# suyashk12/hipgp

Measured on NVIDIA B200. Metric: toeplitz_matvec_GBps_in_pcg_1e6grid, higher is better.
Workload: dtype f32

## Files before the change

### hipgp_b200/csrc/cols_blk_kernel.cuh

```cuda
#pragma once
#include "fast_kernels.cuh"
#include "tma_maps.cuh"

namespace hipgp {

#ifdef HIPGP_EMU
static inline void nbar_sync(int id, int count) { emu::g_named_barrier[id].sync(count); }
static inline void warp_sync_all() {
    const int tid = (int)(threadIdx.x + blockDim.x * (threadIdx.y + blockDim.y * threadIdx.z));
    emu::g_warp_barrier[tid >> 5].wait();
}
#else
__device__ __forceinline__ void nbar_sync(int id, int count) { asm volatile("bar.sync %0, %1;" ::"r"(id), "r"(count) : "memory"); }
__device__ __forceinline__ void warp_sync_all() { __syncwarp(); }
#endif

template <int GS> __device__ __forceinline__ void blk_sync(int b) {
    if (GS == 32) warp_sync_all(); else nbar_sync(1 + b, GS);
}

template <int R, int S, class T>
__device__ __forceinline__ void blk_fill_pairs(TwPair<T>* dst, const cplx<T>* tab, int tid, int nt) {
    for (int i = tid; i < TwPairs<R>::n * S; i += nt) { const int p = i / S; dst[i] = tw_pair_global<R, S, T>(tab, p, i - p * S); }
}
template <int R, int S, bool SM, class T> __device__ __forceinline__ TwPair<T> blk_pair(const cplx<T>* tab, int p, int j) {
    return SM ? reinterpret_cast<const TwPair<T>*>(tab)[p * S + j] : tw_pair_global<R, S, T>(tab, p, j);
}

template <int R, int S, bool SM, class T>
__device__ __forceinline__ void blk_twiddles(cplx<T>* w, const cplx<T>* tab, int j) {
#pragma unroll
    for (int p = 0; p < TwPairs<R>::n; ++p) {
        const TwPair<T> e = blk_pair<R, S, SM, T>(tab, p, j);
        w[2 * p + 1] = e.a;
        if (2 * p + 2 < R) w[2 * p + 2] = e.b;
    }
}

template <int R, int S, bool SM, bool CONJ, int CH, class T>
__device__ __forceinline__ void blk_twiddle_mul(Lane<T>* v, const cplx<T>* tab, int j) {
    constexpr int PC = CH / 2 > 0 ? CH / 2 : 1;
#pragma unroll
    for (int p0 = 0; p0 < TwPairs<R>::n; p0 += PC) {
        TwPair<T> e[PC];
#pragma unroll
        for (int c = 0; c < PC; ++c) if (p0 + c < TwPairs<R>::n) e[c] = blk_pair<R, S, SM, T>(tab, p0 + c, j);
#pragma unroll
        for (int c = 0; c < PC; ++c) if (p0 + c < TwPairs<R>::n) {
            const int r = 2 * (p0 + c) + 1;
            v[r] = CONJ ? lmulc(v[r], e[c].a) : lmul(v[r], e[c].a);
            if (r + 1 < R) v[r + 1] = CONJ ? lmulc(v[r + 1], e[c].b) : lmul(v[r + 1], e[c].b);
        }
#ifndef HIPGP_EMU
        if (p0 + PC < TwPairs<R>::n) asm volatile("" ::: "memory");
#endif
    }
}

template <class T, int NL, int NT, int MINB, int R0, int R1, int R2>
struct ColsBlkCfg {
    using G = TileGeo<T, NL, R0, R1, R2>;
    static constexpr int Ln = G::Ln, BS = Ln / R0, GS = NT / R0;
    static constexpr int IB2 = (BS / R1) * NL, IB3 = (BS / R2) * NL;
    static constexpr bool ok = (NT % R0 == 0) && (GS % 32 == 0) && (GS == 32 || R0 <= 15) && (IB2 % GS == 0) && (IB3 % GS == 0) &&
                               ((IB2 / GS) * R1 <= 16) && ((IB3 / GS) * R2 <= 16) && (BS % R2 == 0);
    static constexpr size_t tw_bytes = 2 * sizeof(cplx<T>) * (size_t)((R0 / 2) * (Ln / R0) + (R1 / 2) * (BS / R1));
    static constexpr size_t side_bytes = (size_t)(Ln + Ln / R2) * NL * 8;
    static constexpr bool tw_smem = (size_t)MINB * (G::smem_bytes() + side_bytes + tw_bytes + 1024) <= 228 * 1024;
    static constexpr size_t smem_bytes = G::smem_bytes() + side_bytes + (tw_smem ? tw_bytes : 0);
};

template <class T, int NL, int NT, int MINB, int R0, int R1, int R2>
__global__ void __launch_bounds__(NT, MINB) cols_blk_kernel(const HIPGP_GRID_CONSTANT ColsParams<T> P, const HIPGP_GRID_CONSTANT ColsTmaMaps maps) {
    using Cfg = ColsBlkCfg<T, NL, NT, MINB, R0, R1, R2>;
    using G = typename Cfg::G;
    constexpr int Ln = G::Ln, RLAST = R2, LPT = LaneInfo<T>::LPT, TBL = NL * LPT, S0 = Ln / R0;
    constexpr int BS = Cfg::BS, GS = Cfg::GS, S1 = BS / R1;
    constexpr bool TWS = Cfg::tw_smem;
    constexpr int TWCH = R0 >= 16 ? 5 : R0;
    static_assert(Cfg::ok, "radix list / tile shape not usable with block-local middle sections");
    constexpr int LEG0 = G::leg(S0), LEG1 = G::leg(S1);
    constexpr int SPEC_LANE = 8;
    constexpr int SIDE_SLOTS = Ln + Ln / RLAST;
    constexpr int SIDE_LANES = SIDE_SLOTS * NL / 2;
    HIPGP_DYN_SMEM(smem_raw);
    Lane<T>* s = reinterpret_cast<Lane<T>*>(smem_raw);
    unsigned char* side = smem_raw + G::smem_bytes();
    const int tid = threadIdx.x;
    if (P.done_flag && *P.done_flag) return;
    const int blk = tid / GS, u = tid - blk * GS;

    const cplx<T>* tw0 = P.f.twst + P.f.twoff[0];
    const cplx<T>* tw1 = P.f.twst + P.f.twoff[1];
    __shared__ unsigned long long s_bar[3];
    const bool tma_in = P.tma_in != 0, tma_spec = P.tma_spec != 0;
    if ((tma_in || tma_spec) && tid == 0) { tma_bar_init(&s_bar[0]); tma_bar_init(&s_bar[1]); warps_bar_init(&s_bar[2], NT / 32); tma_fence_before_issue(); }
    if (tma_in || tma_spec) __syncthreads();
    if (TWS) {
        TwPair<T>* t0 = reinterpret_cast<TwPair<T>*>(side + Cfg::side_bytes);
        TwPair<T>* t1 = t0 + TwPairs<R0>::n * S0;
        blk_fill_pairs<R0, S0, T>(t0, tw0, tid, NT);
        blk_fill_pairs<R1, S1, T>(t1, tw1, tid, NT);
        tw0 = reinterpret_cast<const cplx<T>*>(t0); tw1 = reinterpret_cast<const cplx<T>*>(t1);
        __syncthreads();
    }

    const int mode = P.mode;
    const size_t pitch = (size_t)P.pitch;
    const size_t spitch = P.spec_pitch ? (size_t)P.spec_pitch : (size_t)P.pitch;
    const long ntiles = (long)P.nx * P.ny * P.nz;
    unsigned tile_bz = 0;
    auto tile_origin = [&](long t, long& c0, size_t& ioff, size_t& ooff) {
        const unsigned tt = (unsigned)t, nx = (unsigned)P.nx, ny = (unsigned)P.ny, nz = (unsigned)P.nz;
        unsigned bx, by, bz;
        if (P.batch_fastest) { bz = tt % nz; const unsigned r = tt / nz; bx = r % nx; by = r / nx; }
        else { bx = tt % nx; const unsigned r = tt / nx; by = r % ny; bz = r / ny; }
        c0 = (long)bx * TBL;
        tile_bz = bz;
        ioff = (size_t)by * P.in_ostride + (size_t)bz * P.in_bstride + c0;
        ooff = (size_t)by * P.out_ostride + (size_t)bz * P.out_bstride + c0;
    };
    auto sslot = [](int p) { return p + (p >> G::LOGRL); };
    const bool spec_smem = P.spec_stage != 0;
    const int n_in = P.n_in, n_out = P.n_out;
    const bool stage_in = P.in_stage != 0;
    const bool zero_hi = is_pow2(R0) && n_in <= Ln / 2;
    const bool out_lo = is_pow2(R0) && n_out <= Ln / 2;
    const size_t rstep = (size_t)S0 * pitch;

    auto prefetch_input = [&](long t) {
        long c0; size_t ioff, ooff;
        tile_origin(t, c0, ioff, ooff);
        const long nvalid = P.inner - c0;
        const cplx<T>* in = P.in + ioff;
        constexpr int NIT = (SIDE_LANES + NT - 1) / NT;
        const int total = n_in * NL;
#pragma unroll
        for (int k = 0; k < NIT; ++k) {
            const int w = tid + k * NT;
            const int i = w / NL, lane = w - i * NL;
            if (w < total && (long)lane * LPT < nvalid) cp_async<16>(side + (size_t)w * 16, in + (size_t)i * pitch + lane * LPT);
        }
        cp_async_commit();
    };

    auto issue_input = [&](long t) {
        long c0; size_t ioff, ooff;
        tile_origin(t, c0, ioff, ooff);
        const unsigned box_bytes = (unsigned)P.tma_in_rows * NL * 16u;
        tma_fence_before_issue();
        tma_bar_expect(&s_bar[0], box_bytes * (unsigned)P.tma_in_nbox);
        for (int k = 0; k < P.tma_in_nbox; ++k)
            tma_load_box3(side + (size_t)k * box_bytes, &maps.in, (int)(2 * c0), k * P.tma_in_rows, (int)tile_bz, &s_bar[0]);
    };
    auto stage_next = [&](long tn) {
        if (tn >= ntiles) return;
        if (tma_in) { if (tid == 0) issue_input(tn); }
        else if (stage_in) prefetch_input(tn);
    };

    stage_next((long)blockIdx.x);
    for (unsigned iter = 0;; ++iter) {
        const long t = (long)blockIdx.x + (long)iter * gridDim.x;
        if (t >= ntiles) break;
        const unsigned ph = iter & 1u;
        long c0; size_t ioff, ooff;
        tile_origin(t, c0, ioff, ooff);
        const long nvalid = P.inner - c0;
        const cplx<T>* in = P.in + ioff;
        cplx<T>* out = P.out + ooff;
        if (tma_in) { tma_bar_wait(&s_bar[0], ph, 8, NT); if (mode != CM_FUSED) __syncthreads(); }
        else { cp_async_wait_all(); __syncthreads(); }

        if (mode != CM_INV) {
#pragma unroll 1
            for (int it = tid; it < S0 * NL; it += NT) {
                const int lane = it % NL, j = it / NL;
                const bool ok = (long)lane * LPT < nvalid;
                Lane<T> v[R0];
                if (tma_in) {
                    const Lane<T>* sp = reinterpret_cast<const Lane<T>*>(side) + (j * NL + lane);
#pragma unroll
                    for (int r = 0; r < R0 / 2; ++r) v[r] = sp[r * S0 * NL];
                    lbfly_zero_hi<R0, T>(v);
                } else if (stage_in) {
                    const Lane<T>* sp = reinterpret_cast<const Lane<T>*>(side) + (j * NL + lane);
                    if (zero_hi) {
#pragma unroll
                        for (int r = 0; r < R0 / 2; ++r) v[r] = (ok && j + r * S0 < n_in) ? sp[r * S0 * NL] : lzero<T>();
                        lbfly_zero_hi<R0, T>(v);
                    } else {
#pragma unroll
                        for (int r = 0; r < R0; ++r) v[r] = (ok && j + r * S0 < n_in) ? sp[r * S0 * NL] : lzero<T>();
                        lbfly<R0, false, T>(v);
                    }
                } else {
                    const cplx<T>* gp = in + (size_t)j * pitch + lane * LPT;
                    if (zero_hi) {
#pragma unroll
                        for (int r = 0; r < R0 / 2; ++r) v[r] = (ok && j + r * S0 < n_in) ? lane_from_global(gp + r * rstep) : lzero<T>();
                        lbfly_zero_hi<R0, T>(v);
                    } else {
#pragma unroll
                        for (int r = 0; r < R0; ++r) v[r] = (ok && j + r * S0 < n_in) ? lane_from_global(gp + r * rstep) : lzero<T>();
                        lbfly<R0, false, T>(v);
                    }
                }
                blk_twiddle_mul<R0, S0, TWS, false, TWCH>(v, tw0, j);
                Lane<T>* base = s + (G::slot(j) * NL + lane);
#pragma unroll
                for (int r = 0; r < R0; ++r) base[r * LEG0] = v[r];
            }
            __syncthreads();
            if (!(mode == CM_FUSED && spec_smem)) stage_next(t + gridDim.x);
        }

        const int pb = blk * BS;
        if (mode == CM_FUSED && spec_smem && tma_spec) {
            if (tid == 0) {
                tma_fence_before_issue();
                tma_bar_expect(&s_bar[1], (unsigned)Cfg::side_bytes);
                tma_load_box3(side, &maps.spec, (int)c0, 0, 0, &s_bar[1]);
            }
        } else if (mode == CM_FUSED && spec_smem) {
            const unsigned char* sp = reinterpret_cast<const unsigned char*>(P.spec) + (size_t)c0 * sizeof(T);
            constexpr int ROWB = NL * SPEC_LANE;
            constexpr int CH = ROWB >= 16 ? 16 : 8, NCH = ROWB / CH;
            constexpr int NIT = (BS * NCH + GS - 1) / GS;
#pragma unroll
            for (int k = 0; k < NIT; ++k) {
                const int w = u + k * GS;
                const int p = pb + w / NCH, c = w % NCH;
                if (w < BS * NCH) cp_async<CH>(side + (size_t)sslot(p) * ROWB + c * CH, sp + (size_t)p * spitch * sizeof(T) + c * CH);
            }
            cp_async_commit();
        }
        if (mode != CM_INV) {
            constexpr int NIT = Cfg::IB2 / GS;
            Lane<T> v[NIT][R1];
            cplx<T> w[NIT][R1];
            Lane<T>* base[NIT];
#pragma unroll
            for (int k = 0; k < NIT; ++k) {
                const int q = u + k * GS;
                const int lane = q % NL, j = q / NL;
                base[k] = s + (G::slot(pb + j) * NL + lane);
                blk_twiddles<R1, S1, TWS>(w[k], tw1, j);
#pragma unroll
                for (int r = 0; r < R1; ++r) v[k][r] = base[k][r * LEG1];
            }
#pragma unroll
            for (int k = 0; k < NIT; ++k) {
                lbfly<R1, false, T>(v[k]);
#pragma unroll
                for (int r = 1; r < R1; ++r) v[k][r] = lmul(v[k][r], w[k][r]);
#pragma unroll
                for (int r = 0; r < R1; ++r) base[k][r * LEG1] = v[k][r];
            }
            if (mode == CM_FUSED && spec_smem) {
                if (tma_spec) tma_bar_wait(&s_bar[1], ph, 9, NT);
                else cp_async_wait_all();
            }
            blk_sync<GS>(blk);
        }
        {
            constexpr int NIT = Cfg::IB3 / GS;
#pragma unroll
            for (int k = 0; k < NIT; ++k) {
                const int q = u + k * GS;
                const int lane = q % NL;
                const bool ok = (long)lane * LPT < nvalid;
                const int p0 = pb + (q / NL) * RLAST;
                Lane<T>* base = s + (G::slot(p0) * NL + lane);
                Lane<T> v[RLAST];
                if (mode == CM_INV) {
                    const cplx<T>* gp = in + cols_rowoff<T>(p0, P.pitch, P.in_split_len, P.in_split_stride) + lane * LPT;
#pragma unroll
                    for (int r = 0; r < RLAST; ++r) v[r] = ok ? lane_from_global(gp + r * pitch) : lzero<T>();
                } else {
#pragma unroll
                    for (int r = 0; r < RLAST; ++r) v[r] = base[r * NL];
                    lbfly<RLAST, false, T>(v);
                }
                if (mode == CM_FUSED) {
                    if (spec_smem) {
                        const unsigned char* sp = side + ((size_t)sslot(p0) * NL + lane) * SPEC_LANE;
#pragma unroll
                        for (int r = 0; r < RLAST; ++r) v[r] = lane_spec_smem(v[r], sp + r * NL * SPEC_LANE);
                    } else if (ok) {
                        const size_t sidx = (size_t)p0 * spitch + c0 + lane * LPT;
#pragma unroll
                        for (int r = 0; r < RLAST; ++r) v[r] = lane_spec(v[r], P.spec, P.spec_kind, sidx + (size_t)r * spitch);
                    }
                }
                if (mode == CM_FWD) {
                    if (ok) {
                        cplx<T>* gp = out + cols_rowoff<T>(p0, P.pitch, P.out_split_len, P.out_split_stride) + lane * LPT;
#pragma unroll
                        for (int r = 0; r < RLAST; ++r) lane_to_global(gp + r * pitch, v[r]);
                    }
                } else {
                    lbfly<RLAST, true, T>(v);
#pragma unroll
                    for (int r = 0; r < RLAST; ++r) base[r * NL] = v[r];
                }
            }
        }
        if (mode == CM_FWD) continue;
        const bool early_in = tma_in && mode == CM_FUSED && spec_smem;
        if (early_in) {
            warp_sync_all();
            if (tid == 0) { warps_bar_arrive_and_wait(&s_bar[2], ph, 10, NT / 32); stage_next(t + gridDim.x); }
            else if ((tid & 31) == 0) warps_bar_arrive(&s_bar[2], 10, NT / 32);
        }
        blk_sync<GS>(blk);
        {
            constexpr int NIT = Cfg::IB2 / GS;
            Lane<T> v[NIT][R1];
            cplx<T> w[NIT][R1];
            Lane<T>* base[NIT];
#pragma unroll
            for (int k = 0; k < NIT; ++k) {
                const int q = u + k * GS;
                const int lane = q % NL, j = q / NL;
                base[k] = s + (G::slot(pb + j) * NL + lane);
                blk_twiddles<R1, S1, TWS>(w[k], tw1, j);
#pragma unroll
                for (int r = 0; r < R1; ++r) v[k][r] = base[k][r * LEG1];
            }
#pragma unroll
            for (int k = 0; k < NIT; ++k) {
#pragma unroll
                for (int r = 1; r < R1; ++r) v[k][r] = lmulc(v[k][r], w[k][r]);
                lbfly<R1, true, T>(v[k]);
#pragma unroll
                for (int r = 0; r < R1; ++r) base[k][r * LEG1] = v[k][r];
            }
        }
        __syncthreads();
        if (mode == CM_FUSED && spec_smem && !early_in) stage_next(t + gridDim.x);
        {
#pragma unroll 1
            for (int it = tid; it < S0 * NL; it += NT) {
                const int lane = it % NL, j = it / NL;
                const bool ok = (long)lane * LPT < nvalid;
                const Lane<T>* base = s + (G::slot(j) * NL + lane);
                Lane<T> v[R0];
#pragma unroll
                for (int r = 0; r < R0; ++r) v[r] = base[r * LEG0];
                blk_twiddle_mul<R0, S0, TWS, true, TWCH>(v, tw0, j);
                cplx<T>* gp = out + (size_t)((unsigned)j * (unsigned)P.pitch + (unsigned)(lane * LPT));
                const unsigned rs = (unsigned)S0 * (unsigned)P.pitch;
                if (out_lo) {
                    lbfly<R0, true, T>(v);
                    if (ok) {
#pragma unroll
                        for (int r = 0; r < R0 / 2; ++r) if (j + r * S0 < n_out) lane_to_global(gp + (size_t)((unsigned)r * rs), v[r]);
                    }
                } else {
                    lbfly<R0, true, T>(v);
                    if (ok) {
#pragma unroll
                        for (int r = 0; r < R0; ++r) if (j + r * S0 < n_out) lane_to_global(gp + (size_t)((unsigned)r * rs), v[r]);
                    }
                }
            }
        }
    }
}

}
```

### hipgp_b200/csrc/conv_kernels.cuh

```cuda
#pragma once
#include "fft_engine.cuh"

namespace hipgp {

enum RowsFwdMode { RF_PLAIN = 0, RF_PUPDATE = 1, RF_XRUPDATE = 2, RF_SELFDOT = 3 };
enum RowsInvMode { RI_PLAIN = 0, RI_DOT = 1 };
enum DotKind { DOT_PAP = 0, DOT_ZR = 1, DOT_RR = 2 };
enum ColsMode { CM_FWD = 0, CM_INV = 1, CM_FUSED = 2 };
enum SpecKind { SPEC_NONE = 0, SPEC_REAL = 1, SPEC_CPLX = 2, SPEC_CPLX_CONJ = 3 };

struct PcgDev {
    double* zr;
    double* zr_prev;
    double* pAp;
    double* rr;
    const double* rr_all;
    double* partial;
    unsigned* row_cnt;
    unsigned* rhs_cnt;
    int* flags;
    double tol;
    int B;
    int cg_mode;
};

template <class T> __device__ __forceinline__ T warp_sum(T v) {
#pragma unroll
    for (int o = 16; o > 0; o >>= 1) v += __shfl_xor_sync(0xffffffffu, v, o);
    return v;
}

__device__ __forceinline__ void pcg_finalize(const PcgDev& st, int kind, long g0, long g1, int nrows, int tid, int nthreads) {
    __shared__ unsigned s_last;
    __shared__ double s_red[32];
    const int b0 = (int)(g0 / nrows), b1 = (int)((g1 - 1) / nrows);
    for (int b = b0; b <= b1; ++b) {
        const long lo = g0 > (long)b * nrows ? g0 : (long)b * nrows;
        const long hi = g1 < (long)(b + 1) * nrows ? g1 : (long)(b + 1) * nrows;
        __syncthreads();
        if (tid == 0) {
            __threadfence();
            const unsigned done = atomicAdd(st.row_cnt + b, (unsigned)(hi - lo)) + (unsigned)(hi - lo);
            s_last = (done == (unsigned)nrows);
        }
        __syncthreads();
        if (!s_last) continue;
        __threadfence();
        double acc = 0.0;
        const volatile double* part = st.partial + (long)b * nrows;
        for (int i = tid; i < nrows; i += nthreads) acc += part[i];
        acc = warp_sum(acc);
        if ((tid & 31) == 0) s_red[tid >> 5] = acc;
        __syncthreads();
        if (tid < 32) {
            double v = tid < (nthreads >> 5) ? s_red[tid] : 0.0;
            v = warp_sum(v);
            if (tid == 0) {
                st.row_cnt[b] = 0;
                if (kind == DOT_PAP) st.pAp[b] = v;
                else if (kind == DOT_ZR) { st.zr_prev[b] = st.zr[b]; st.zr[b] = v; }
                else {
                    st.rr[b] = v;
                    if (st.cg_mode) { st.zr_prev[b] = st.zr[b]; st.zr[b] = v; }
                }
                __threadfence();
                if (kind == DOT_RR) {
                    const unsigned nb = atomicAdd(st.rhs_cnt, 1u) + 1u;
                    if (nb == (unsigned)st.B) {
                        __threadfence();
                        bool all = true;
                        const volatile double* rr = st.rr_all ? st.rr_all : st.rr;
                        for (int i = 0; i < st.B; ++i) all = all && (sqrt(rr[i]) < st.tol);
                        st.rhs_cnt[0] = 0;
                        st.flags[1] += 1;
                        st.flags[2] = 0;
                        if (all) st.flags[0] = 1;
                    }
                }
            }
        }
    }
}

template <class T>
struct RowsParams {
    const T* in;
    T* out;
    T* v0;
    T* v1;
    const T* v2;
    cplx<T>* W;
    long total_rows;
    int nrows;
    int n_real;
    int L, H;
    long W_pitch;
    int W_rows;
    LineFft<T> f;
    const cplx<T>* twL;
    const cplx<T>* twLp;
    const int* part;
    const int* pairq;
    const int* pairs; const cplx<T>* pairw; int npair0;
    const int* quadq; const cplx<T>* quadw; int nquad;
    int RB, RBP;
    int mode, dot_kind, do_fft;
    int vec_ok;
    int vec16_ok;
    int tma_ok;
    int tma_op;
    const void* spec; int spec_kind;
    PcgDev st;
};

template <class T>
__global__ void __launch_bounds__(256) rows_fwd_kernel(RowsParams<T> P) {
    HIPGP_DYN_SMEM(smem_raw);
    cplx<T>* s = reinterpret_cast<cplx<T>*>(smem_raw);
    const int tid = threadIdx.x, nthreads = blockDim.x;
    const int warp = tid >> 5, lane = tid & 31, nwarps = nthreads >> 5;
    if (P.mode != RF_PLAIN && P.st.flags[0]) return;
    const long g0 = (long)blockIdx.x * P.RB;
    const long g1 = g0 + P.RB < P.total_rows ? g0 + P.RB : P.total_rows;
    const int nl = (int)(g1 - g0);
    const int H = P.H, RBP = P.RBP, n = P.n_real;

    for (int line = warp; line < P.RB; line += nwarps) {
        if (line >= nl) {
            if (P.do_fft) for (int k = lane; k < H; k += 32) s[(size_t)k * RBP + line] = mk<T>(0, 0);
            continue;
        }
        const long g = g0 + line;
        const int b = (int)(g / P.nrows);
        const size_t off = (size_t)g * n;
        T acc = 0;
        T coef = 0;
        bool first = false;
        if (P.mode == RF_PUPDATE) {
            first = P.st.flags[2] != 0;
            coef = first ? (T)0 : (T)(P.st.zr[b] / P.st.zr_prev[b]);
        } else if (P.mode == RF_XRUPDATE) {
            coef = (T)(P.st.zr[b] / P.st.pAp[b]);
        }
        for (int k = lane; k < H; k += 32) {
            T e[2];
#pragma unroll
            for (int h = 0; h < 2; ++h) {
                const int i = 2 * k + h;
                T val = 0;
                if (i < n) {
                    if (P.mode == RF_PLAIN) {
                        val = P.in[off + i];
                    } else if (P.mode == RF_PUPDATE) {
                        const T z = P.in[off + i];
                        val = first ? z : z + coef * P.v0[off + i];
                        P.v0[off + i] = val;
                    } else if (P.mode == RF_SELFDOT) {
                        val = P.in[off + i];
                        acc += val * val;
                    } else {
                        const T pv = P.v2[off + i];
                        P.v1[off + i] = P.v1[off + i] + coef * pv;
                        val = P.v0[off + i] - coef * P.in[off + i];
                        P.v0[off + i] = val;
                        acc += val * val;
                    }
                }
                e[h] = val;
            }
            if (P.do_fft) s[(size_t)k * RBP + line] = mk<T>(e[0], e[1]);
        }
        if (P.mode == RF_XRUPDATE || P.mode == RF_SELFDOT) {
            const double tot = warp_sum((double)acc);
            if (lane == 0) P.st.partial[g] = tot;
        }
    }
    if (P.mode == RF_XRUPDATE) pcg_finalize(P.st, DOT_RR, g0, g1, P.nrows, tid, nthreads);
    if (P.mode == RF_SELFDOT) pcg_finalize(P.st, DOT_ZR, g0, g1, P.nrows, tid, nthreads);
    if (!P.do_fft) return;
    __syncthreads();

    fft_forward(s, RBP, P.RB, P.f, tid, nthreads);

    for (int w = tid; w < H * P.RB; w += nthreads) {
        const int line = w % P.RB, p = w / P.RB;
        const int k = P.f.rev[p];
        if (k == 0) {
            const cplx<T> z = s[line];
            s[line] = mk<T>((T)2 * (z.x + z.y), 0);
            s[(size_t)H * RBP + line] = mk<T>((T)2 * (z.x - z.y), 0);
        } else {
            const int k2 = H - k;
            if (k <= k2) {
                const int p2 = P.f.pos[k2];
                const cplx<T> a = s[(size_t)p * RBP + line], c = conj(s[(size_t)p2 * RBP + line]);
                const cplx<T> E = a + c;
                const cplx<T> d = a - c;
                const cplx<T> O = mk<T>(d.y, -d.x);
                const cplx<T> t = P.twL[k] * O;
                s[(size_t)p * RBP + line] = E + t;
                if (k != k2) s[(size_t)p2 * RBP + line] = conj(E - t);
            }
        }
    }
    __syncthreads();

    for (int line = warp; line < nl; line += nwarps) {
        const long g = g0 + line;
        cplx<T>* dst = P.W + ((size_t)(g / P.nrows) * P.W_rows + (g % P.nrows)) * P.W_pitch;
        for (int q = lane; q <= H; q += 32) dst[q] = s[(size_t)q * RBP + line];
    }
}

template <class T>
__device__ __forceinline__ cplx<T> apply_spec(cplx<T> v, const void* spec, int kind, size_t idx) {
    if (kind == SPEC_REAL) return v * reinterpret_cast<const T*>(spec)[idx];
    const cplx<T> sv = reinterpret_cast<const cplx<T>*>(spec)[idx];
    return kind == SPEC_CPLX ? v * sv : mulc(v, sv);
}

template <class T>
__global__ void __launch_bounds__(256) rows_inv_kernel(RowsParams<T> P) {
    HIPGP_DYN_SMEM(smem_raw);
    cplx<T>* s = reinterpret_cast<cplx<T>*>(smem_raw);
    const int tid = threadIdx.x, nthreads = blockDim.x;
    const int warp = tid >> 5, lane = tid & 31, nwarps = nthreads >> 5;
    if (P.mode != RI_PLAIN && P.st.flags[0]) return;
    const long g0 = (long)blockIdx.x * P.RB;
    const long g1 = g0 + P.RB < P.total_rows ? g0 + P.RB : P.total_rows;
    const int nl = (int)(g1 - g0);
    const int H = P.H, RBP = P.RBP, n = P.n_real;

    for (int line = warp; line < P.RB; line += nwarps) {
        if (line >= nl) {
            for (int q = lane; q <= H; q += 32) s[(size_t)q * RBP + line] = mk<T>(0, 0);
            continue;
        }
        const long g = g0 + line;
        const cplx<T>* src = P.W + ((size_t)(g / P.nrows) * P.W_rows + (g % P.nrows)) * P.W_pitch;
        for (int q = lane; q <= H; q += 32) {
            cplx<T> v = src[q];
            if (P.spec_kind != SPEC_NONE) v = apply_spec(v, P.spec, P.spec_kind, (size_t)q);
            s[(size_t)q * RBP + line] = v;
        }
    }
    __syncthreads();

    for (int w = tid; w < H * P.RB; w += nthreads) {
        const int line = w % P.RB, p = w / P.RB;
        const int k = P.f.rev[p];
        if (k == 0) {
            const T y0 = s[line].x, yh = s[(size_t)H * RBP + line].x;
            s[line] = mk<T>(y0 + yh, y0 - yh);
        } else {
            const int k2 = H - k;
            if (k <= k2) {
                const int p2 = P.f.pos[k2];
                const cplx<T> a = s[(size_t)p * RBP + line], c = conj(s[(size_t)p2 * RBP + line]);
                const cplx<T> E = a + c;
                const cplx<T> O = mulc(a - c, P.twL[k]);
                const cplx<T> iO = mk<T>(-O.y, O.x);
                s[(size_t)p * RBP + line] = E + iO;
                if (k != k2) s[(size_t)p2 * RBP + line] = conj(E - iO);
            }
        }
    }
    __syncthreads();

    fft_inverse(s, RBP, P.RB, P.f, tid, nthreads);

    for (int line = warp; line < nl; line += nwarps) {
        const long g = g0 + line;
        const size_t off = (size_t)g * n;
        T acc = 0;
        for (int k = lane; k < H; k += 32) {
            const cplx<T> z = s[(size_t)k * RBP + line];
            const int i = 2 * k;
            if (i < n) { P.out[off + i] = z.x; if (P.mode == RI_DOT) acc += z.x * P.v0[off + i]; }
            if (i + 1 < n) { P.out[off + i + 1] = z.y; if (P.mode == RI_DOT) acc += z.y * P.v0[off + i + 1]; }
        }
        if (P.mode == RI_DOT) {
            const double tot = warp_sum((double)acc);
            if (lane == 0) P.st.partial[g] = tot;
        }
    }
    if (P.mode == RI_DOT) pcg_finalize(P.st, P.dot_kind, g0, g1, P.nrows, tid, nthreads);
}

template <class T>
struct ColsParams {
    const cplx<T>* in;
    cplx<T>* out;
    int n_in, n_out;
    long inner;
    long pitch;
    long in_ostride, in_bstride, out_ostride, out_bstride;
    LineFft<T> f;
    int TB, TBP;
    int mode;
    const void* spec; int spec_kind;
    long spec_pitch;
    int spec_stage;
    int in_stage;
    int nx, ny, nz;
    int tma_in, tma_in_rows, tma_in_nbox;
    int tma_spec;
    int batch_fastest;
    const int* done_flag;
    int out_split_len; long out_split_stride;
    int in_split_len; long in_split_stride;
};
template <class T> __device__ __forceinline__ size_t cols_rowoff(int i, long pitch, int split_len, long split_stride) {
    return split_len ? (size_t)(i / split_len) * split_stride + (size_t)(i % split_len) * pitch : (size_t)i * pitch;
}

template <class T>
__global__ void __launch_bounds__(512) cols_pass_kernel(ColsParams<T> P) {
    HIPGP_DYN_SMEM(smem_raw);
    cplx<T>* s = reinterpret_cast<cplx<T>*>(smem_raw);
    const int tid = threadIdx.x, nthreads = blockDim.x;
    if (P.done_flag && *P.done_flag) return;
    const long c0 = (long)blockIdx.x * P.TB;
    const int nc = (int)(P.inner - c0 < P.TB ? P.inner - c0 : P.TB);
    const int L = P.f.Ln, TB = P.TB, TBP = P.TBP;
    const cplx<T>* in = P.in + (size_t)blockIdx.y * P.in_ostride + (size_t)blockIdx.z * P.in_bstride + c0;
    cplx<T>* out = P.out + (size_t)blockIdx.y * P.out_ostride + (size_t)blockIdx.z * P.out_bstride + c0;

    const int rows_in = P.mode == CM_INV ? L : P.n_in;
    for (int w = tid; w < L * TB; w += nthreads) {
        const int c = w % TB, i = w / TB;
        cplx<T> v = mk<T>(0, 0);
        if (i < rows_in && c < nc) v = in[cols_rowoff<T>(i, P.pitch, P.in_split_len, P.in_split_stride) + c];
        s[(size_t)i * TBP + c] = v;
    }
    __syncthreads();

    if (P.mode != CM_INV) fft_forward(s, TBP, TB, P.f, tid, nthreads);
    if (P.mode == CM_FUSED) {
        for (int w = tid; w < L * TB; w += nthreads) {
            const int c = w % TB, i = w / TB;
            if (c < nc) s[(size_t)i * TBP + c] = apply_spec(s[(size_t)i * TBP + c], P.spec, P.spec_kind, (size_t)i * (P.spec_pitch ? P.spec_pitch : P.pitch) + c0 + c);
        }
        __syncthreads();
    }
    if (P.mode != CM_FWD) fft_inverse(s, TBP, TB, P.f, tid, nthreads);

    const int rows_out = P.mode == CM_FWD ? L : P.n_out;
    for (int w = tid; w < rows_out * TB; w += nthreads) {
        const int c = w % TB, i = w / TB;
        if (c < nc) out[cols_rowoff<T>(i, P.pitch, P.out_split_len, P.out_split_stride) + c] = s[(size_t)i * TBP + c];
    }
}


}
```

### hipgp_b200/csrc/cuda_emu.h

```cpp
#pragma once
#ifdef HIPGP_EMU
#include <algorithm>
#include <atomic>
#include <cmath>
#include <condition_variable>
#include <cstdint>
#include <cstdio>
#include <cstdlib>
#include <cstring>
#include <functional>
#include <mutex>
#include <thread>
#include <vector>

#define __global__
#define __device__
#define __host__
#define __forceinline__ inline
#define __restrict__
#define __launch_bounds__(...)
#define __shared__ static
#define __align__(n) alignas(n)

struct uint3e { unsigned x, y, z; };
struct dim3 {
    unsigned x, y, z;
    dim3(unsigned x_ = 1, unsigned y_ = 1, unsigned z_ = 1) : x(x_), y(y_), z(z_) {}
};
struct float2 { float x, y; };
struct double2 { double x, y; };
static inline float2 make_float2(float a, float b) { return float2{a, b}; }
static inline double2 make_double2(double a, double b) { return double2{a, b}; }

typedef void* cudaStream_t;
typedef void* cudaEvent_t;
typedef int cudaError_t;
enum { cudaSuccess = 0 };
enum cudaMemcpyKind { cudaMemcpyHostToDevice, cudaMemcpyDeviceToHost, cudaMemcpyDeviceToDevice, cudaMemcpyDefault };

namespace emu {
struct Barrier {
    std::mutex mu;
    std::condition_variable cv;
    int expected = 0, arrived = 0;
    unsigned long gen = 0;
    void reset(int n) { expected = n; arrived = 0; }
    void wait() {
        std::unique_lock<std::mutex> lk(mu);
        unsigned long g = gen;
        if (++arrived >= expected) { arrived = 0; ++gen; cv.notify_all(); return; }
        cv.wait(lk, [&] { return gen != g; });
    }
    void drop() {
        std::unique_lock<std::mutex> lk(mu);
        --expected;
        if (expected > 0 && arrived >= expected) { arrived = 0; ++gen; cv.notify_all(); }
    }
};
struct NamedBarrier {
    std::mutex mu;
    std::condition_variable cv;
    int arrived = 0;
    unsigned long gen = 0;
    void reset() { arrived = 0; }
    void arrive(int expected) {
        std::unique_lock<std::mutex> lk(mu);
        if (++arrived >= expected) { arrived = 0; ++gen; cv.notify_all(); }
    }
    void sync(int expected) {
        std::unique_lock<std::mutex> lk(mu);
        const unsigned long g = gen;
        if (++arrived >= expected) { arrived = 0; ++gen; cv.notify_all(); return; }
        cv.wait(lk, [&] { return gen != g; });
    }
};
extern NamedBarrier g_named_barrier[16];
extern thread_local dim3 t_threadIdx, t_blockIdx;
extern dim3 g_blockDim, g_gridDim;
extern Barrier g_block_barrier;
extern Barrier g_warp_barrier[64];
extern unsigned char* g_dyn_smem;
extern double g_shfl_scratch[64][32][2];

template <class F>
void launch(dim3 grid, dim3 block, size_t smem, F&& body) {
    const int T = (int)(block.x * block.y * block.z);
    g_blockDim = block; g_gridDim = grid;
    std::vector<unsigned char> dyn(smem + 64);
    g_dyn_smem = dyn.data() + (64 - ((uintptr_t)dyn.data() & 63)) % 64;
    Barrier start, finish;
    const long nblocks = (long)grid.x * grid.y * grid.z;
    start.reset(T); finish.reset(T);
    auto worker = [&](int t) {
        t_threadIdx = dim3(t % block.x, (t / block.x) % block.y, t / (block.x * block.y));
        for (long b = 0; b < nblocks; ++b) {
            t_blockIdx = dim3((unsigned)(b % grid.x), (unsigned)((b / grid.x) % grid.y), (unsigned)(b / ((long)grid.x * grid.y)));
            if (t == 0) {
                g_block_barrier.reset(T);
                for (int w = 0; w < 64; ++w) g_warp_barrier[w].reset(32);
                for (int w = 0; w < 16; ++w) g_named_barrier[w].reset();
            }
            start.wait();
            body();
            g_block_barrier.drop();
            finish.wait();
        }
    };
    std::vector<std::thread> th;
    th.reserve(T);
    for (int t = 1; t < T; ++t) th.emplace_back(worker, t);
    worker(0);
    for (auto& x : th) x.join();
    g_dyn_smem = nullptr;
}
}

#define threadIdx emu::t_threadIdx
#define blockIdx emu::t_blockIdx
#define blockDim emu::g_blockDim
#define gridDim emu::g_gridDim
static inline void __syncthreads() { emu::g_block_barrier.wait(); }
static inline void __syncwarp(unsigned = 0xffffffffu) {}
static inline void __threadfence() { std::atomic_thread_fence(std::memory_order_seq_cst); }

template <class T>
static inline T __shfl_xor_sync(unsigned, T v, int lanemask) {
    const int tid = (int)(threadIdx.x + blockDim.x * (threadIdx.y + blockDim.y * threadIdx.z));
    const int w = tid >> 5, l = tid & 31;
    static_assert(sizeof(T) <= 16, "shfl payload");
    std::memcpy(emu::g_shfl_scratch[w][l], &v, sizeof(T));
    emu::g_warp_barrier[w].wait();
    T r;
    std::memcpy(&r, emu::g_shfl_scratch[w][l ^ lanemask], sizeof(T));
    emu::g_warp_barrier[w].wait();
    return r;
}
template <class T>
static inline T __shfl_down_sync(unsigned, T v, int delta) {
    const int tid = (int)(threadIdx.x + blockDim.x * (threadIdx.y + blockDim.y * threadIdx.z));
    const int w = tid >> 5, l = tid & 31;
    std::memcpy(emu::g_shfl_scratch[w][l], &v, sizeof(T));
    emu::g_warp_barrier[w].wait();
    T r;
    std::memcpy(&r, emu::g_shfl_scratch[w][(l + delta) < 32 ? l + delta : l], sizeof(T));
    emu::g_warp_barrier[w].wait();
    return r;
}
static inline unsigned atomicAdd(unsigned* p, unsigned v) { return __atomic_fetch_add(p, v, __ATOMIC_SEQ_CST); }
static inline int atomicAdd(int* p, int v) { return __atomic_fetch_add(p, v, __ATOMIC_SEQ_CST); }
static inline unsigned atomicInc_emu(unsigned* p) { return __atomic_fetch_add(p, 1u, __ATOMIC_SEQ_CST); }
template <class T> static inline T __ldg(const T* p) { return *p; }
static inline int __popc(int x) { return __builtin_popcount((unsigned)x); }
static inline void sincospi(double x, double* s, double* c) { *s = std::sin(M_PI * x); *c = std::cos(M_PI * x); }
static inline double cospi(double x) { return std::cos(M_PI * x); }
static inline double rsqrt(double x) { return 1.0 / std::sqrt(x); }
static inline float rsqrtf(float x) { return 1.0f / std::sqrt(x); }

static inline cudaError_t cudaMalloc(void** p, size_t n) { *p = std::malloc(n ? n : 1); return *p ? 0 : 2; }
static inline cudaError_t cudaFree(void* p) { std::free(p); return 0; }
static inline cudaError_t cudaMallocHost(void** p, size_t n) { return cudaMalloc(p, n); }
static inline cudaError_t cudaFreeHost(void* p) { return cudaFree(p); }
static inline cudaError_t cudaMemcpyAsync(void* d, const void* s, size_t n, cudaMemcpyKind, cudaStream_t) { std::memcpy(d, s, n); return 0; }
static inline cudaError_t cudaMemcpy(void* d, const void* s, size_t n, cudaMemcpyKind) { std::memcpy(d, s, n); return 0; }
static inline cudaError_t cudaMemsetAsync(void* d, int v, size_t n, cudaStream_t) { std::memset(d, v, n); return 0; }
static inline cudaError_t cudaMemset(void* d, int v, size_t n) { std::memset(d, v, n); return 0; }
static inline cudaError_t cudaStreamSynchronize(cudaStream_t) { return 0; }
static inline cudaError_t cudaDeviceSynchronize() { return 0; }
static inline cudaError_t cudaGetLastError() { return 0; }
static inline cudaError_t cudaSetDevice(int) { return 0; }
static inline cudaError_t cudaGetDevice(int* d) { *d = 0; return 0; }
static inline const char* cudaGetErrorString(cudaError_t) { return "emu"; }

#define HIPGP_DYN_SMEM(name) unsigned char* name = emu::g_dyn_smem
#define HIPGP_LAUNCH(kernel, grid, block, smem, stream, ...) \
    emu::launch((grid), (block), (smem), [&]() { kernel(__VA_ARGS__); })
#define HIPGP_SET_MAX_SMEM(kernel, bytes) ((void)0)

#else
#include <cuda_runtime.h>
#include <cstdint>
#include <cstdio>
#include <cstdlib>
#include <cstring>
#include <cmath>
#include <algorithm>
#include <vector>

#define HIPGP_DYN_SMEM(name) extern __shared__ __align__(128) unsigned char name[]
#define HIPGP_LAUNCH(kernel, grid, block, smem, stream, ...) \
    kernel<<<(grid), (block), (smem), (stream)>>>(__VA_ARGS__)
#define HIPGP_SET_MAX_SMEM(kernel, bytes) \
    cudaFuncSetAttribute(kernel, cudaFuncAttributeMaxDynamicSharedMemorySize, (int)(bytes))
#endif
```

### hipgp_b200/csrc/fast_kernels.cuh

```cuda
#pragma once
#include "lane_fft.cuh"

namespace hipgp {

template <class T> __device__ __forceinline__ void ld2(const T* p, bool vec, T& a, T& b, bool ok0, bool ok1) {
    if (vec && ok1) { const cplx<T> t = ld_stream(reinterpret_cast<const cplx<T>*>(p)); a = t.x; b = t.y; }
    else { a = ok0 ? ld_stream(p) : (T)0; b = ok1 ? ld_stream(p + 1) : (T)0; }
}
template <class T> __device__ __forceinline__ void st2(T* p, bool vec, T a, T b, bool ok0, bool ok1) {
    if (vec && ok1) { st_stream(reinterpret_cast<cplx<T>*>(p), mk<T>(a, b)); }
    else { if (ok0) st_stream(p, a); if (ok1) st_stream(p + 1, b); }
}

__device__ __forceinline__ double team_sum(double v, int tw) {
    for (int o = tw >> 1; o > 0; o >>= 1) v += __shfl_xor_sync(0xffffffffu, v, o);
    return v;
}

__device__ __forceinline__ Lane<float> lane_spec(Lane<float> v, const void* spec, int kind, size_t idx) {
    if (kind == SPEC_REAL) {
        const cplx<float> sv = ld_stream(reinterpret_cast<const cplx<float>*>(reinterpret_cast<const float*>(spec) + idx));
        return lmul_real2(v, sv.x, sv.y);
    }
    const cplx<float>* sp = reinterpret_cast<const cplx<float>*>(spec) + idx;
    const cplx<float> w0 = ld_stream(sp), w1 = ld_stream(sp + 1);
    return kind == SPEC_CPLX ? lmul_cplx2<false>(v, w0, w1) : lmul_cplx2<true>(v, w0, w1);
}
__device__ __forceinline__ Lane<double> lane_spec(Lane<double> v, const void* spec, int kind, size_t idx) {
    if (kind == SPEC_REAL) return lscale(v, ld_stream(reinterpret_cast<const double*>(spec) + idx));
    const cplx<double> w = ld_stream(reinterpret_cast<const cplx<double>*>(spec) + idx);
    return kind == SPEC_CPLX ? lmul(v, w) : lmulc(v, w);
}
__device__ __forceinline__ Lane<float> lane_spec_smem(Lane<float> v, const void* p) {
    const float2 s2 = *reinterpret_cast<const float2*>(p);
    Lane<float> r; r.re = __fmul2_rn(v.re, s2); r.im = __fmul2_rn(v.im, s2); return r;
}
__device__ __forceinline__ Lane<double> lane_spec_smem(Lane<double> v, const void* p) { return lscale(v, *reinterpret_cast<const double*>(p)); }

template <class T, int NL, int NT, int MINB, int R0, int... Rs>
__global__ void __launch_bounds__(NT, MINB) cols_fast_kernel(ColsParams<T> P) {
    using G = TileGeo<T, NL, R0, Rs...>;
    constexpr int Ln = G::Ln, NST = G::NST, RLAST = G::RLAST, LPT = LaneInfo<T>::LPT, TBL = NL * LPT, S0 = Ln / R0;
    HIPGP_DYN_SMEM(smem_raw);
    Lane<T>* s = reinterpret_cast<Lane<T>*>(smem_raw);
    const int tid = threadIdx.x;
    if (P.done_flag && *P.done_flag) return;
    const int mode = P.mode;
    const size_t pitch = (size_t)P.pitch;
    const size_t spitch = P.spec_pitch ? (size_t)P.spec_pitch : (size_t)P.pitch;
    const long ntiles = (long)P.nx * P.ny * P.nz;
    auto tile_origin = [&](long t, long& c0, size_t& ioff, size_t& ooff) {
        long bx, by, bz;
        if (P.batch_fastest) { bz = t % P.nz; const long r = t / P.nz; bx = r % P.nx; by = r / P.nx; }
        else { bx = t % P.nx; const long r = t / P.nx; by = r % P.ny; bz = r / P.ny; }
        c0 = bx * TBL;
        ioff = (size_t)by * P.in_ostride + (size_t)bz * P.in_bstride + c0;
        ooff = (size_t)by * P.out_ostride + (size_t)bz * P.out_bstride + c0;
    };

    if constexpr (NST == 1) {
        for (long t = blockIdx.x; t < ntiles; t += gridDim.x) {
            long c0; size_t ioff, ooff;
            tile_origin(t, c0, ioff, ooff);
            const long nvalid = P.inner - c0;
            const cplx<T>* in = P.in + ioff;
            cplx<T>* out = P.out + ooff;
            for (int lane = tid; lane < NL; lane += NT) {
                if ((long)lane * LPT >= nvalid) continue;
                const int rows_in = mode == CM_INV ? Ln : P.n_in;
                const int rows_out = mode == CM_FWD ? Ln : P.n_out;
                Lane<T> v[R0];
#pragma unroll
                for (int r = 0; r < R0; ++r)
                    v[r] = r < rows_in ? lane_from_global(in + cols_rowoff<T>(r, P.pitch, P.in_split_len, P.in_split_stride) + lane * LPT) : lzero<T>();
                if (mode != CM_INV) lbfly<R0, false, T>(v);
                if (mode == CM_FUSED) {
#pragma unroll
                    for (int r = 0; r < R0; ++r) v[r] = lane_spec(v[r], P.spec, P.spec_kind, (size_t)r * spitch + c0 + lane * LPT);
                }
                if (mode != CM_FWD) lbfly<R0, true, T>(v);
#pragma unroll
                for (int r = 0; r < R0; ++r)
                    if (r < rows_out) lane_to_global(out + cols_rowoff<T>(r, P.pitch, P.out_split_len, P.out_split_stride) + lane * LPT, v[r]);
            }
        }
        return;
    } else {
        constexpr int LEG0 = G::leg(S0);
        constexpr int SPEC_LANE = 8;
        constexpr int SIDE_SLOTS = Ln + Ln / RLAST;
        constexpr int SIDE_LANES = SIDE_SLOTS * NL / 2;
        unsigned char* side = smem_raw + G::smem_bytes();
        auto sslot = [](int p) { return p + (p >> G::LOGRL); };
        const cplx<T>* tw0 = P.f.twst + P.f.twoff[0];
        const bool spec_smem = P.spec_stage != 0;
        const int n_in = P.n_in, n_out = P.n_out;
        const bool stage_in = P.in_stage != 0;
        const bool zero_hi = is_pow2(R0) && n_in <= Ln / 2;
        const bool out_lo = is_pow2(R0) && n_out <= Ln / 2;
        const size_t rstep = (size_t)S0 * pitch;

        auto prefetch_input = [&](long t) {
            long c0; size_t ioff, ooff;
            tile_origin(t, c0, ioff, ooff);
            const long nvalid = P.inner - c0;
            const cplx<T>* in = P.in + ioff;
            constexpr int NIT = (SIDE_LANES + NT - 1) / NT;
            const int total = n_in * NL;
#pragma unroll
            for (int k = 0; k < NIT; ++k) {
                const int w = tid + k * NT;
                const int i = w / NL, lane = w - i * NL;
                if (w < total && (long)lane * LPT < nvalid) cp_async<16>(side + (size_t)w * 16, in + (size_t)i * pitch + lane * LPT);
            }
            cp_async_commit();
        };

        long t = blockIdx.x;
        if (stage_in && t < ntiles) prefetch_input(t);
        for (; t < ntiles; t += gridDim.x) {
            long c0; size_t ioff, ooff;
            tile_origin(t, c0, ioff, ooff);
            const long nvalid = P.inner - c0;
            const cplx<T>* in = P.in + ioff;
            cplx<T>* out = P.out + ooff;
            cp_async_wait_all();
            __syncthreads();

            if (mode != CM_INV) {
#pragma unroll 1
                for (int it = tid; it < S0 * NL; it += NT) {
                    const int lane = it % NL, j = it / NL;
                    const bool ok = (long)lane * LPT < nvalid;
                    cplx<T> w[R0];
                    lane_twiddles<R0, S0>(w, tw0, j);
                    Lane<T> v[R0];
                    if (stage_in) {
                        const Lane<T>* sp = reinterpret_cast<const Lane<T>*>(side) + (j * NL + lane);
                        if (zero_hi) {
#pragma unroll
                            for (int r = 0; r < R0 / 2; ++r) v[r] = (ok && j + r * S0 < n_in) ? sp[r * S0 * NL] : lzero<T>();
                            lbfly_zero_hi<R0, T>(v);
                        } else {
#pragma unroll
                            for (int r = 0; r < R0; ++r) v[r] = (ok && j + r * S0 < n_in) ? sp[r * S0 * NL] : lzero<T>();
                            lbfly<R0, false, T>(v);
                        }
                    } else {
                        const cplx<T>* gp = in + (size_t)j * pitch + lane * LPT;
                        if (zero_hi) {
#pragma unroll
                            for (int r = 0; r < R0 / 2; ++r) v[r] = (ok && j + r * S0 < n_in) ? lane_from_global(gp + r * rstep) : lzero<T>();
                            lbfly_zero_hi<R0, T>(v);
                        } else {
#pragma unroll
                            for (int r = 0; r < R0; ++r) v[r] = (ok && j + r * S0 < n_in) ? lane_from_global(gp + r * rstep) : lzero<T>();
                            lbfly<R0, false, T>(v);
                        }
                    }
#pragma unroll
                    for (int r = 1; r < R0; ++r) v[r] = lmul(v[r], w[r]);
                    Lane<T>* base = s + (G::slot(j) * NL + lane);
#pragma unroll
                    for (int r = 0; r < R0; ++r) base[r * LEG0] = v[r];
                }
                __syncthreads();
                if (spec_smem) {
                    const unsigned char* sp = reinterpret_cast<const unsigned char*>(P.spec) + (size_t)c0 * sizeof(T);
                    constexpr int ROWB = NL * SPEC_LANE;
                    constexpr int CH = ROWB >= 16 ? 16 : 8, NCH = ROWB / CH;
                    constexpr int NIT = (Ln * NCH + NT - 1) / NT;
#pragma unroll
                    for (int k = 0; k < NIT; ++k) {
                        const int w = tid + k * NT;
                        const int p = w / NCH, c = w - p * NCH;
                        if (w < Ln * NCH) cp_async<CH>(side + (size_t)sslot(p) * ROWB + c * CH, sp + (size_t)p * spitch * sizeof(T) + c * CH);
                    }
                    cp_async_commit();
                }
                LaneMidFwd<G, T, NL, NT, Ln / R0, 1, Rs...>::run(s, P.f, tid);
                if (spec_smem) { cp_async_wait_all(); __syncthreads(); }
            }

            {
#pragma unroll 2
                for (int it = tid; it < (Ln / RLAST) * NL; it += NT) {
                    const int lane = it % NL, bf = it / NL;
                    const bool ok = (long)lane * LPT < nvalid;
                    const int p0 = bf * RLAST;
                    Lane<T>* base = s + (G::slot(p0) * NL + lane);
                    Lane<T> v[RLAST];
                    if (mode == CM_INV) {
                        const cplx<T>* gp = in + cols_rowoff<T>(p0, P.pitch, P.in_split_len, P.in_split_stride) + lane * LPT;
#pragma unroll
                        for (int r = 0; r < RLAST; ++r) v[r] = ok ? lane_from_global(gp + r * pitch) : lzero<T>();
                    } else {
#pragma unroll
                        for (int r = 0; r < RLAST; ++r) v[r] = base[r * NL];
                        lbfly<RLAST, false, T>(v);
                    }
                    if (mode == CM_FUSED) {
                        if (spec_smem) {
                            const unsigned char* sp = side + ((size_t)sslot(p0) * NL + lane) * SPEC_LANE;
#pragma unroll
                            for (int r = 0; r < RLAST; ++r) v[r] = lane_spec_smem(v[r], sp + r * NL * SPEC_LANE);
                        } else if (ok) {
                            const size_t sidx = (size_t)p0 * spitch + c0 + lane * LPT;
#pragma unroll
                            for (int r = 0; r < RLAST; ++r) v[r] = lane_spec(v[r], P.spec, P.spec_kind, sidx + (size_t)r * spitch);
                        }
                    }
                    if (mode == CM_FWD) {
                        if (ok) {
                            cplx<T>* gp = out + cols_rowoff<T>(p0, P.pitch, P.out_split_len, P.out_split_stride) + lane * LPT;
#pragma unroll
                            for (int r = 0; r < RLAST; ++r) lane_to_global(gp + r * pitch, v[r]);
                        }
                    } else {
                        lbfly<RLAST, true, T>(v);
#pragma unroll
                        for (int r = 0; r < RLAST; ++r) base[r * NL] = v[r];
                    }
                }
                __syncthreads();
            }
            if (stage_in && t + gridDim.x < ntiles) prefetch_input(t + gridDim.x);
            if (mode == CM_FWD) continue;

            LaneMidInv<G, T, NL, NT, Ln / R0, 1, Rs...>::run(s, P.f, tid);
            {
#pragma unroll 1
                for (int it = tid; it < S0 * NL; it += NT) {
                    const int lane = it % NL, j = it / NL;
                    const bool ok = (long)lane * LPT < nvalid;
                    cplx<T> w[R0];
                    lane_twiddles<R0, S0>(w, tw0, j);
                    const Lane<T>* base = s + (G::slot(j) * NL + lane);
                    Lane<T> v[R0];
#pragma unroll
                    for (int r = 0; r < R0; ++r) v[r] = base[r * LEG0];
#pragma unroll
                    for (int r = 1; r < R0; ++r) v[r] = lmulc(v[r], w[r]);
                    cplx<T>* gp = out + (size_t)j * pitch + lane * LPT;
                    lbfly<R0, true, T>(v);
                    if (ok) {
                        if (out_lo) {
#pragma unroll
                            for (int r = 0; r < R0 / 2; ++r) if (j + r * S0 < n_out) lane_to_global(gp + r * rstep, v[r]);
                        } else {
#pragma unroll
                            for (int r = 0; r < R0; ++r) if (j + r * S0 < n_out) lane_to_global(gp + r * rstep, v[r]);
                        }
                    }
                }
            }
        }
    }
}

struct __align__(8) QuadIdx { int a, b; };

template <class T, int NL, int NT, int MINB, int R0, int... Rs>
__global__ void __launch_bounds__(NT, MINB) rows_fwd_fast_kernel(RowsParams<T> P) {
    using G = TileGeo<T, NL, R0, Rs...>;
    constexpr int H = G::Ln, NST = G::NST, RLAST = G::RLAST, LPT = LaneInfo<T>::LPT, NROW = NL * LPT, S0 = H / R0;
    constexpr int LEG0 = G::leg(NST > 1 ? S0 : 1);
    HIPGP_DYN_SMEM(smem_raw);
    Lane<T>* s = reinterpret_cast<Lane<T>*>(smem_raw);
    const int tid = threadIdx.x;
    if (P.mode != RF_PLAIN && P.st.flags[0]) return;
    const long g0 = (long)blockIdx.x * NROW;
    const long g1 = g0 + NROW < P.total_rows ? g0 + NROW : P.total_rows;
    const int nl = (int)(g1 - g0);
    const int n = P.n_real;
    const int mode = P.mode;
    const bool vec = ((n & 1) == 0) && P.vec_ok;
    const bool first_it = (mode == RF_PUPDATE) && (P.st.flags[2] != 0);
    const bool want_dot = (mode == RF_XRUPDATE || mode == RF_SELFDOT);
    __shared__ T s_coef[32];
    __shared__ long s_wbase[32];
    __shared__ double s_part[32];
    if (tid < NROW && tid < nl) {
        const long gr = g0 + tid;
        const long b = gr / P.nrows;
        s_wbase[tid] = (b * P.W_rows + (gr - b * P.nrows)) * P.W_pitch;
        T coef = 0;
        if (mode == RF_PUPDATE) coef = first_it ? (T)0 : (T)(P.st.zr[b] / P.st.zr_prev[b]);
        else if (mode == RF_XRUPDATE) coef = (T)(P.st.zr[b] / P.st.pAp[b]);
        s_coef[tid] = coef;
    }
    __syncthreads();

    const int SROW = (n + 3) & ~3;
    T* side = reinterpret_cast<T*>(smem_raw + G::smem_bytes());
    bool streamed = false;
#ifndef HIPGP_EMU
    bool bulk_store_pending = false;
    if (P.tma_ok && P.vec16_ok && SROW == n && (mode == RF_PLAIN || mode == RF_SELFDOT || P.tma_op)) {
        constexpr int CH = 16 / (int)sizeof(T);
        __shared__ __align__(8) unsigned long long s_mbar;
        const unsigned bytes = (unsigned)((size_t)nl * n * sizeof(T));
        const size_t goff = (size_t)g0 * n;
        T* bufA = reinterpret_cast<T*>(smem_raw);
        T* bufB = bufA + (size_t)NROW * SROW;
        const bool two = mode == RF_PUPDATE && !first_it, three = mode == RF_XRUPDATE;
        if (tid == 0) { mbar_init(&s_mbar, 1); fence_proxy_async(); }
        __syncthreads();
        if (tid == 0) {
            mbar_arrive_expect_tx(&s_mbar, bytes * (three ? 3u : (two ? 2u : 1u)));
            bulk_g2s(side, P.in + goff, bytes, &s_mbar);
            if (two) bulk_g2s(bufA, (const T*)P.v0 + goff, bytes, &s_mbar);
            if (three) { bulk_g2s(bufA, (const T*)P.v0 + goff, bytes, &s_mbar); bulk_g2s(bufB, P.v2 + goff, bytes, &s_mbar); }
        }
        constexpr int NW = NT / 32, WPR = NW > NROW ? NW / NROW : 1;
        constexpr int tws = WPR > 1 ? 32 : (H / CH >= 32 ? 32 : (H / CH >= 16 ? 16 : (H / CH >= 8 ? 8 : 4)));
        constexpr int rpw = 32 / tws, TW = WPR > 1 ? 32 * WPR : tws, rstep = WPR > 1 ? NW / WPR : NW * rpw;
        const int warp = tid >> 5, l32 = tid & 31;
        const int ln = WPR > 1 ? l32 + 32 * (warp % WPR) : l32 % tws;
        const int nch = n / CH;
        mbar_wait(&s_mbar, 0);
        if (mode != RF_PLAIN && !(mode == RF_PUPDATE && first_it)) {
            for (int rbase = WPR > 1 ? warp / WPR : warp * rpw; rbase < nl; rbase += rstep) {
                const int row = rbase + (WPR > 1 ? 0 : l32 / tws);
                const bool ractive = row < nl;
                double acc = 0.0;
                if (ractive) {
                    T* srow = side + (size_t)row * SROW;
                    const T* arow = bufA + (size_t)row * SROW;
                    const T* brow = bufB + (size_t)row * SROW;
                    const size_t off = goff + (size_t)row * n;
                    const T coef = s_coef[row];
                    if (three) {
                        constexpr int BS = 4;
                        for (int cb = ln; cb < nch; cb += TW * BS) {
                            Vec16<T> xv[BS];
#pragma unroll
                            for (int k = 0; k < BS; ++k) { const int c = cb + TW * k; if (c < nch) xv[k] = ldv_stream((const T*)P.v1 + off + (size_t)c * CH); }
#pragma unroll
                            for (int k = 0; k < BS; ++k) {
                                const int c = cb + TW * k;
                                if (c < nch) {
                                    Vec16<T> q = *reinterpret_cast<const Vec16<T>*>(srow + c * CH);
                                    const Vec16<T> rv = *reinterpret_cast<const Vec16<T>*>(arow + c * CH);
                                    const Vec16<T> pv = *reinterpret_cast<const Vec16<T>*>(brow + c * CH);
#pragma unroll
                                    for (int e = 0; e < CH; ++e) { xv[k].v[e] = xv[k].v[e] + coef * pv.v[e]; q.v[e] = rv.v[e] - coef * q.v[e]; acc += (double)(q.v[e] * q.v[e]); }
                                    stv_stream(P.v1 + off + (size_t)c * CH, xv[k]);
                                    *reinterpret_cast<Vec16<T>*>(srow + c * CH) = q;
                                }
                            }
                        }
                    } else if (two) {
                        for (int c = ln; c < nch; c += TW) {
                            Vec16<T> z = *reinterpret_cast<const Vec16<T>*>(srow + c * CH);
                            const Vec16<T> pv = *reinterpret_cast<const Vec16<T>*>(arow + c * CH);
#pragma unroll
                            for (int e = 0; e < CH; ++e) z.v[e] = z.v[e] + coef * pv.v[e];
                            *reinterpret_cast<Vec16<T>*>(srow + c * CH) = z;
                        }
                    } else {
                        for (int c = ln; c < nch; c += TW) {
                            const Vec16<T> z = *reinterpret_cast<const Vec16<T>*>(srow + c * CH);
#pragma unroll
                            for (int e = 0; e < CH; ++e) acc += (double)(z.v[e] * z.v[e]);
                        }
                    }
                }
                if (want_dot) {
                    acc = team_sum(acc, WPR > 1 ? 32 : tws);
                    if (ractive && (WPR > 1 ? l32 == 0 : ln == 0)) s_part[row * WPR + warp % WPR] = acc;
                }
            }
        }
        if (mode == RF_PUPDATE || mode == RF_XRUPDATE) {
            fence_proxy_async();
            __syncthreads();
            if (tid == 0) {
                asm volatile("cp.async.bulk.global.shared::cta.bulk_group [%0], [%1], %2;" ::"l"(P.v0 + goff), "r"((unsigned)__cvta_generic_to_shared(side)), "r"(bytes) : "memory");
                asm volatile("cp.async.bulk.commit_group;" ::: "memory");
            }
            bulk_store_pending = true;
        }
        if (want_dot) {
            __syncthreads();
            if (tid < nl) { double a = 0.0; for (int k = 0; k < WPR; ++k) a += s_part[tid * WPR + k]; P.st.partial[g0 + tid] = a; }
        }
        streamed = true;
    }
#endif
    if (!streamed) {
        constexpr int CH = 16 / (int)sizeof(T);
        constexpr int NW = NT / 32, WPR = NW > NROW ? NW / NROW : 1;
        const bool chunked = P.vec16_ok && (n % CH == 0);
        constexpr int tws = WPR > 1 ? 32 : (H / CH >= 32 ? 32 : (H / CH >= 16 ? 16 : (H / CH >= 8 ? 8 : 4)));
        constexpr int rpw = 32 / tws;
        constexpr int TW = WPR > 1 ? 32 * WPR : tws;
        const int warp = tid >> 5, l32 = tid & 31;
        const int ln = WPR > 1 ? l32 + 32 * (warp % WPR) : l32 % tws;
        constexpr int rstep = WPR > 1 ? NW / WPR : NW * rpw;
        for (int rbase = WPR > 1 ? warp / WPR : warp * rpw; rbase < nl; rbase += rstep) {
            const int row = rbase + (WPR > 1 ? 0 : l32 / tws);
            const bool ractive = row < nl;
            T* srow = side + (size_t)(ractive ? row : 0) * SROW;
            const size_t off = (size_t)(g0 + (ractive ? row : 0)) * n;
            const T coef = s_coef[ractive ? row : 0];
            double acc = 0.0;
            if (!ractive) {
            } else if (chunked) {
                const int nch = n / CH;
                auto finish = [&](int c, Vec16<T> a) {
                    if (want_dot) {
#pragma unroll
                        for (int k = 0; k < CH; ++k) acc += (double)(a.v[k] * a.v[k]);
                    }
                    *reinterpret_cast<Vec16<T>*>(srow + c * CH) = a;
                };
#define HIPGP_PIPE(LOAD, PROC)                                                                              \
                {                                                                                           \
                    const int step = TW * BS;                                                               \
                    int cb = ln;                                                                            \
                    LOAD(0, cb);                                                                            \
                    for (; cb < nch; cb += 2 * step) {                                                      \
                        if (cb + step < nch) { LOAD(1, cb + step); }                                        \
                        PROC(0, cb);                                                                        \
                        if (cb + 2 * step < nch) { LOAD(0, cb + 2 * step); }                                \
                        if (cb + step < nch) { PROC(1, cb + step); }                                        \
                    }                                                                                       \
                }
                if (mode == RF_XRUPDATE) {
                    constexpr int BS = 1;
                    Vec16<T> a[2][BS], pv[2][BS], xv[2][BS], rv[2][BS];
#define HIPGP_LD(S, CB)                                                                                     \
                    _Pragma("unroll") for (int k = 0; k < BS; ++k) {                                        \
                        const int c = (CB) + TW * k;                                                        \
                        if (c < nch) {                                                                      \
                            const size_t o = off + (size_t)c * CH;                                          \
                            a[S][k] = ldv_stream(P.in + o); pv[S][k] = ldv_stream(P.v2 + o);                \
                            xv[S][k] = ldv_stream((const T*)P.v1 + o); rv[S][k] = ldv_stream((const T*)P.v0 + o); \
                        }                                                                                   \
                    }
#define HIPGP_PR(S, CB)                                                                                     \
                    _Pragma("unroll") for (int k = 0; k < BS; ++k) {                                        \
                        const int c = (CB) + TW * k;                                                        \
                        if (c < nch) {                                                                      \
                            const size_t o = off + (size_t)c * CH;                                          \
                            _Pragma("unroll") for (int e = 0; e < CH; ++e) {                                \
                                xv[S][k].v[e] = xv[S][k].v[e] + coef * pv[S][k].v[e];                       \
                                a[S][k].v[e] = rv[S][k].v[e] - coef * a[S][k].v[e];                         \
                            }                                                                               \
                            stv_stream(P.v1 + o, xv[S][k]);                                                 \
                            stv_stream(P.v0 + o, a[S][k]);                                                  \
                            finish(c, a[S][k]);                                                             \
                        }                                                                                   \
                    }
                    HIPGP_PIPE(HIPGP_LD, HIPGP_PR)
#undef HIPGP_LD
#undef HIPGP_PR
                } else if (mode == RF_PUPDATE && !first_it) {
                    constexpr int BS = 2;
                    Vec16<T> a[2][BS], pv[2][BS];
#define HIPGP_LD(S, CB)                                                                                     \
                    _Pragma("unroll") for (int k = 0; k < BS; ++k) {                                        \
                        const int c = (CB) + TW * k;                                                        \
                        if (c < nch) { const size_t o = off + (size_t)c * CH; a[S][k] = ldv_stream(P.in + o); pv[S][k] = ldv_stream((const T*)P.v0 + o); } \
                    }
#define HIPGP_PR(S, CB)                                                                                     \
                    _Pragma("unroll") for (int k = 0; k < BS; ++k) {                                        \
                        const int c = (CB) + TW * k;                                                        \
                        if (c < nch) {                                                                      \
                            _Pragma("unroll") for (int e = 0; e < CH; ++e) a[S][k].v[e] = a[S][k].v[e] + coef * pv[S][k].v[e]; \
                            stv_stream(P.v0 + off + (size_t)c * CH, a[S][k]);                               \
                            finish(c, a[S][k]);                                                             \
                        }                                                                                   \
                    }
                    HIPGP_PIPE(HIPGP_LD, HIPGP_PR)
#undef HIPGP_LD
#undef HIPGP_PR
                } else {
                    constexpr int BS = 4;
                    const bool wr = mode == RF_PUPDATE;
                    Vec16<T> a[2][BS];
#define HIPGP_LD(S, CB)                                                                                     \
                    _Pragma("unroll") for (int k = 0; k < BS; ++k) { const int c = (CB) + TW * k; if (c < nch) a[S][k] = ldv_stream(P.in + off + (size_t)c * CH); }
#define HIPGP_PR(S, CB)                                                                                     \
                    _Pragma("unroll") for (int k = 0; k < BS; ++k) {                                        \
                        const int c = (CB) + TW * k;                                                        \
                        if (c < nch) { if (wr) stv_stream(P.v0 + off + (size_t)c * CH, a[S][k]); finish(c, a[S][k]); } \
                    }
                    HIPGP_PIPE(HIPGP_LD, HIPGP_PR)
#undef HIPGP_LD
#undef HIPGP_PR
                }
#undef HIPGP_PIPE
            } else {
                for (int i = ln; i < n; i += TW) {
                    const size_t o = off + i;
                    T a = ld_stream(P.in + o);
                    if (mode == RF_PUPDATE) {
                        if (!first_it) a = a + coef * ld_stream((const T*)P.v0 + o);
                        st_stream(P.v0 + o, a);
                    } else if (mode == RF_XRUPDATE) {
                        const T pv = ld_stream(P.v2 + o);
                        st_stream(P.v1 + o, ld_stream((const T*)P.v1 + o) + coef * pv);
                        a = ld_stream((const T*)P.v0 + o) - coef * a;
                        st_stream(P.v0 + o, a);
                    }
                    if (want_dot) acc += (double)(a * a);
                    srow[i] = a;
                }
            }
            if (ractive) for (int i = n + ln; i < SROW; i += TW) srow[i] = (T)0;
            if (want_dot) {
                acc = team_sum(acc, WPR > 1 ? 32 : tws);
                if (ractive && (WPR > 1 ? l32 == 0 : ln == 0)) s_part[row * WPR + warp % WPR] = acc;
            }
        }
        if (want_dot) {
            __syncthreads();
            if (tid < nl) { double a = 0.0; for (int k = 0; k < WPR; ++k) a += s_part[tid * WPR + k]; P.st.partial[g0 + tid] = a; }
        }
    }
    __syncthreads();
    if (want_dot) pcg_finalize(P.st, mode == RF_XRUPDATE ? DOT_RR : DOT_ZR, g0, g1, P.nrows, tid, NT);

    {
        const bool zero_hi = is_pow2(R0) && R0 > 1 && (n + 1) / 2 <= H / 2;
        const cplx<T>* tw0 = P.f.twst + P.f.twoff[0];
#pragma unroll 1
        for (int it = tid; it < S0 * NL; it += NT) {
            const int lane = it % NL, j = it / NL;
            cplx<T> w[R0];
            if (NST > 1) lane_twiddles<R0, S0>(w, tw0, j);
            const T* srow0 = side + (size_t)(lane * LPT) * SROW;
            const T* srow1 = side + (size_t)(lane * LPT + LPT - 1) * SROW;
            const bool ok0 = lane * LPT < nl, ok1 = lane * LPT + LPT - 1 < nl;
            auto elem = [&](int r) -> Lane<T> {
                const int i = 2 * (j + r * S0);
                const bool in_row = i < SROW;
                const cplx<T> e0 = (ok0 && in_row) ? *reinterpret_cast<const cplx<T>*>(srow0 + i) : mk<T>(0, 0);
                const cplx<T> e1 = (LPT == 2 && ok1 && in_row) ? *reinterpret_cast<const cplx<T>*>(srow1 + i) : mk<T>(0, 0);
                return lane_make(e0, e1);
            };
            Lane<T> v[R0];
            if (zero_hi) {
#pragma unroll
                for (int r = 0; r < R0 / 2; ++r) v[r] = elem(r);
                lbfly_zero_hi<R0, T>(v);
            } else {
#pragma unroll
                for (int r = 0; r < R0; ++r) v[r] = elem(r);
                lbfly<R0, false, T>(v);
            }
            if (NST > 1) {
#pragma unroll
                for (int r = 1; r < R0; ++r) v[r] = lmul(v[r], w[r]);
            }
            Lane<T>* base = s + (G::slot(j) * NL + lane);
#pragma unroll
            for (int r = 0; r < R0; ++r) base[r * LEG0] = v[r];
        }
    }
    __syncthreads();

    if constexpr (NST > 1) {
        LaneMidFwd<G, T, NL, NT, H / R0, 1, Rs...>::run(s, P.f, tid);
        lane_stage<G, T, NL, NT, RLAST, RLAST, false>(s, P.f.twst, tid);
        __syncthreads();
    }

    constexpr int NPAIR0 = NST > 1 ? RLAST / 2 + 1 : H / 2 + 1;
    constexpr int NQUAD = NST > 1 ? (H - RLAST) / 4 : 0;
#pragma unroll 1
    for (int it = tid; it < NPAIR0 * NL; it += NT) {
        const int lane = it % NL, pi = it / NL;
        const QuadIdx pq = reinterpret_cast<const QuadIdx*>(P.pairs)[pi];
        const int q = pq.a, q2 = pq.b;
        Lane<T> Xa, Xb;
        bool two;
        if (q == 0) {
            const Lane<T> z = s[lane];
            Lane<T> zs; zs.re = z.im; zs.im = z.re;
            Xa = lscale(z + zs, (T)2); Xb = lscale(z - zs, (T)2);
            Xa.im = lzero<T>().im; Xb.im = lzero<T>().im;
            two = true;
        } else {
            const cplx<T> wq = ldg_c(P.pairw + pi);
            const Lane<T> a = s[G::slot(q) * NL + lane], c = lconj(s[G::slot(q2) * NL + lane]);
            const Lane<T> E = a + c;
            const Lane<T> t = lmul(lmi<false>(a - c), wq);
            Xa = E + t; Xb = lconj(E - t);
            two = q2 != q;
        }
#pragma unroll
        for (int l = 0; l < LPT; ++l) {
            const int row = lane * LPT + l;
            if (row < nl) {
                cplx<T>* dst = P.W + s_wbase[row];
                WRow<T>::store1(dst, q, lane_get(Xa, l));
                if (two) WRow<T>::store1(dst, q2, lane_get(Xb, l));
            }
        }
    }
    if constexpr (NQUAD > 0) {
        constexpr int QIT = (NQUAD * NL + NT - 1) / NT;
        QuadIdx qq[QIT]; cplx<T> wa[QIT], wa1[QIT];
#pragma unroll
        for (int k = 0; k < QIT; ++k) {
            const int it = tid + k * NT, qi = it / NL;
            if (it < NQUAD * NL) { qq[k] = reinterpret_cast<const QuadIdx*>(P.quadq)[qi]; wa[k] = ldg_c(P.quadw + 2 * qi); wa1[k] = ldg_c(P.quadw + 2 * qi + 1); }
        }
#pragma unroll
        for (int k = 0; k < QIT; ++k) {
            const int it = tid + k * NT, lane = it % NL;
            if (it < NQUAD * NL) {
                const Lane<T>* pa = s + (G::slot(qq[k].a) * NL + lane);
                const Lane<T>* pb = s + (G::slot(qq[k].b) * NL + lane);
                const Lane<T> za = pa[0], za1 = pa[NL], zb = pb[0], zb1 = pb[NL];
                Lane<T> c = lconj(zb1);
                Lane<T> E = za + c;
                Lane<T> t = lmul(lmi<false>(za - c), wa[k]);
                const Lane<T> Xa = E + t, Xb1 = lconj(E - t);
                c = lconj(zb);
                E = za1 + c;
                t = lmul(lmi<false>(za1 - c), wa1[k]);
                const Lane<T> Xa1 = E + t, Xb = lconj(E - t);
                const bool self = qq[k].a == qq[k].b;
#pragma unroll
                for (int l = 0; l < LPT; ++l) {
                    const int row = lane * LPT + l;
                    if (row < nl) {
                        cplx<T>* dst = P.W + s_wbase[row];
                        if (self) WRow<T>::store2(dst, qq[k].a, lane_get(Xa, l), lane_get(Xb1, l));
                        else { WRow<T>::store2(dst, qq[k].a, lane_get(Xa, l), lane_get(Xa1, l)); WRow<T>::store2(dst, qq[k].b, lane_get(Xb, l), lane_get(Xb1, l)); }
                    }
                }
            }
        }
    }
#ifndef HIPGP_EMU
    if (bulk_store_pending && tid == 0) asm volatile("cp.async.bulk.wait_group.read 0;" ::: "memory");
#endif
}

template <class T, int NL, int NT, int MINB, int R0, int... Rs>
__global__ void __launch_bounds__(NT, MINB) rows_inv_fast_kernel(RowsParams<T> P) {
    using G = TileGeo<T, NL, R0, Rs...>;
    constexpr int H = G::Ln, NST = G::NST, RLAST = G::RLAST, LPT = LaneInfo<T>::LPT, NROW = NL * LPT, S0 = H / R0;
    constexpr int LEG0 = G::leg(NST > 1 ? S0 : 1);
    HIPGP_DYN_SMEM(smem_raw);
    Lane<T>* s = reinterpret_cast<Lane<T>*>(smem_raw);
    const int tid = threadIdx.x;
    if (P.mode != RI_PLAIN && P.st.flags[0]) return;
    const long g0 = (long)blockIdx.x * NROW;
    const long g1 = g0 + NROW < P.total_rows ? g0 + NROW : P.total_rows;
    const int nl = (int)(g1 - g0);
    const int n = P.n_real;

    __shared__ long s_wbase[32];
    __shared__ double s_part[32];
    if (tid < NROW && tid < nl) {
        const long gr = g0 + tid;
        const long b = gr / P.nrows;
        s_wbase[tid] = (b * P.W_rows + (gr - b * P.nrows)) * P.W_pitch;
    }
    __syncthreads();

    const int spec_kind = P.spec_kind;
    constexpr int NPAIR0 = NST > 1 ? RLAST / 2 + 1 : H / 2 + 1;
    constexpr int NQUAD = NST > 1 ? (H - RLAST) / 4 : 0;
#pragma unroll 1
    for (int it = tid; it < NPAIR0 * NL; it += NT) {
        const int lane = it % NL, pi = it / NL;
        const QuadIdx pq = reinterpret_cast<const QuadIdx*>(P.pairs)[pi];
        const int q = pq.a, q2 = pq.b;
        const cplx<T> wq = ldg_c(P.pairw + pi);
        cplx<T> ya[LPT], yc[LPT];
#pragma unroll
        for (int l = 0; l < LPT; ++l) {
            const int row = lane * LPT + l;
            ya[l] = mk<T>(0, 0); yc[l] = mk<T>(0, 0);
            if (row < nl) {
                const cplx<T>* src = P.W + s_wbase[row];
                ya[l] = WRow<T>::load1(src, q); yc[l] = WRow<T>::load1(src, q2);
                if (spec_kind != SPEC_NONE) { ya[l] = apply_spec(ya[l], P.spec, spec_kind, (size_t)q); yc[l] = apply_spec(yc[l], P.spec, spec_kind, (size_t)q2); }
            }
        }
        const Lane<T> a = lane_make(ya[0], ya[LPT - 1]);
        Lane<T> c = lane_make(yc[0], yc[LPT - 1]);
        if (q == 0) {
            Lane<T> z; z.re = (a + c).re; z.im = (a - c).re;
            s[lane] = z;
        } else {
            c = lconj(c);
            const Lane<T> E = a + c;
            const Lane<T> iO = lmi<true>(lmulc(a - c, wq));
            s[G::slot(q) * NL + lane] = E + iO;
            if (q2 != q) s[G::slot(q2) * NL + lane] = lconj(E - iO);
        }
    }
    if constexpr (NQUAD > 0) {
        constexpr int QIT = (NQUAD * NL + NT - 1) / NT;
        QuadIdx qq[QIT]; cplx<T> wa[QIT], wa1[QIT];
        cplx<T> ya[QIT][LPT], ya1[QIT][LPT], yb[QIT][LPT], yb1[QIT][LPT];
#pragma unroll
        for (int k = 0; k < QIT; ++k) {
            int it = tid + k * NT;
            it = it < NQUAD * NL ? it : NQUAD * NL - 1;
            const int qi = it / NL;
            qq[k] = reinterpret_cast<const QuadIdx*>(P.quadq)[qi]; wa[k] = ldg_c(P.quadw + 2 * qi); wa1[k] = ldg_c(P.quadw + 2 * qi + 1);
        }
#pragma unroll
        for (int k = 0; k < QIT; ++k) {
            int it = tid + k * NT;
            it = it < NQUAD * NL ? it : NQUAD * NL - 1;
            const int lane = it % NL;
#pragma unroll
            for (int l = 0; l < LPT; ++l) {
                const int row = lane * LPT + l;
                const cplx<T>* src = P.W + s_wbase[row < nl ? row : nl - 1];
                WRow<T>::load2(src, qq[k].a, ya[k][l], ya1[k][l]);
                WRow<T>::load2(src, qq[k].b, yb[k][l], yb1[k][l]);
            }
        }
#pragma unroll
        for (int k = 0; k < QIT; ++k) {
            const int it = tid + k * NT, lane = it % NL;
            if (it < NQUAD * NL) {
                const bool self = qq[k].a == qq[k].b;
                if (spec_kind != SPEC_NONE) {
#pragma unroll
                    for (int l = 0; l < LPT; ++l) {
                        ya[k][l] = apply_spec(ya[k][l], P.spec, spec_kind, (size_t)qq[k].a); ya1[k][l] = apply_spec(ya1[k][l], P.spec, spec_kind, (size_t)qq[k].a + 1);
                        yb[k][l] = apply_spec(yb[k][l], P.spec, spec_kind, (size_t)qq[k].b); yb1[k][l] = apply_spec(yb1[k][l], P.spec, spec_kind, (size_t)qq[k].b + 1);
                    }
                }
                const Lane<T> A = lane_make(ya[k][0], ya[k][LPT - 1]), A1 = lane_make(ya1[k][0], ya1[k][LPT - 1]);
                const Lane<T> Bn = lane_make(yb[k][0], yb[k][LPT - 1]), B1 = lane_make(yb1[k][0], yb1[k][LPT - 1]);
                Lane<T>* pa = s + (G::slot(qq[k].a) * NL + lane);
                Lane<T>* pb = s + (G::slot(qq[k].b) * NL + lane);
                Lane<T> c = lconj(B1);
                Lane<T> E = A + c;
                Lane<T> iO = lmi<true>(lmulc(A - c, wa[k]));
                pa[0] = E + iO;
                pb[NL] = lconj(E - iO);
                if (!self) {
                    c = lconj(Bn);
                    E = A1 + c;
                    iO = lmi<true>(lmulc(A1 - c, wa1[k]));
                    pa[NL] = E + iO;
                    pb[0] = lconj(E - iO);
                }
            }
        }
    }
    __syncthreads();

    if constexpr (NST > 1) {
        lane_stage<G, T, NL, NT, RLAST, RLAST, true>(s, P.f.twst, tid);
        __syncthreads();
        LaneMidInv<G, T, NL, NT, H / R0, 1, Rs...>::run(s, P.f, tid);
    }

    const int SROW = (n + 3) & ~3;
    T* side = reinterpret_cast<T*>(smem_raw + G::smem_bytes());
    const bool want_dot = P.mode == RI_DOT;
    {
        const bool out_lo = is_pow2(R0) && R0 > 1 && (n + 1) / 2 <= H / 2;
        const cplx<T>* tw0 = P.f.twst + P.f.twoff[0];
#pragma unroll 1
        for (int it = tid; it < S0 * NL; it += NT) {
            const int lane = it % NL, j = it / NL;
            cplx<T> w[R0];
            if (NST > 1) lane_twiddles<R0, S0>(w, tw0, j);
            const Lane<T>* base = s + (G::slot(j) * NL + lane);
            Lane<T> v[R0];
#pragma unroll
            for (int r = 0; r < R0; ++r) v[r] = base[r * LEG0];
            if (NST > 1) {
#pragma unroll
                for (int r = 1; r < R0; ++r) v[r] = lmulc(v[r], w[r]);
            }
            lbfly<R0, true, T>(v);
            T* srow0 = side + (size_t)(lane * LPT) * SROW;
            T* srow1 = side + (size_t)(lane * LPT + LPT - 1) * SROW;
            auto put = [&](int r) {
                const int i = 2 * (j + r * S0);
                if (i < SROW) {
                    *reinterpret_cast<cplx<T>*>(srow0 + i) = lane_get(v[r], 0);
                    if (LPT == 2) *reinterpret_cast<cplx<T>*>(srow1 + i) = lane_get(v[r], LPT - 1);
                }
            };
            if (out_lo) {
#pragma unroll
                for (int r = 0; r < R0 / 2; ++r) put(r);
            } else {
#pragma unroll
                for (int r = 0; r < R0; ++r) put(r);
            }
        }
    }
#ifndef HIPGP_EMU
    const bool tma_any = P.tma_ok && P.vec16_ok && SROW == n;
    const bool tma_out = !want_dot && tma_any;
    const bool tma_dot = want_dot && tma_any;
    if (tma_any) fence_proxy_async();
#else
    const bool tma_out = false, tma_dot = false;
#endif
    __syncthreads();
#ifndef HIPGP_EMU
    if (tma_out) {
        if (tid == 0) bulk_s2g(P.out + (size_t)g0 * n, side, (unsigned)((size_t)nl * n * sizeof(T)));
        return;
    }
    if (tma_dot && tid == 0) bulk_s2g_issue(P.out + (size_t)g0 * n, side, (unsigned)((size_t)nl * n * sizeof(T)));
#endif
    {
        constexpr int CH = 16 / (int)sizeof(T);
        constexpr int NW = NT / 32, WPR = NW > NROW ? NW / NROW : 1;
        const bool chunked = P.vec16_ok && (n % CH == 0);
        constexpr int tws = WPR > 1 ? 32 : (H / CH >= 32 ? 32 : (H / CH >= 16 ? 16 : (H / CH >= 8 ? 8 : 4)));
        constexpr int rpw = 32 / tws;
        constexpr int TW = WPR > 1 ? 32 * WPR : tws;
        const int warp = tid >> 5, l32 = tid & 31;
        const int ln = WPR > 1 ? l32 + 32 * (warp % WPR) : l32 % tws;
        constexpr int rstep = WPR > 1 ? NW / WPR : NW * rpw;
        for (int rbase = WPR > 1 ? warp / WPR : warp * rpw; rbase < nl; rbase += rstep) {
            const int row = rbase + (WPR > 1 ? 0 : l32 / tws);
            const bool ractive = row < nl;
            const T* srow = side + (size_t)(ractive ? row : 0) * SROW;
            const size_t off = (size_t)(g0 + (ractive ? row : 0)) * n;
            double acc = 0.0;
            if (!ractive) {
            } else if (chunked) {
                const int nch = n / CH;
                constexpr int BS = 8;
                for (int cb = ln; cb < nch; cb += TW * BS) {
                    Vec16<T> ov[BS];
                    if (want_dot) {
#pragma unroll
                        for (int k = 0; k < BS; ++k) { const int c = cb + TW * k; if (c < nch) ov[k] = ldv_stream((const T*)P.v0 + off + (size_t)c * CH); }
                    }
#pragma unroll
                    for (int k = 0; k < BS; ++k) {
                        const int c = cb + TW * k;
                        if (c < nch) {
                            const Vec16<T> y = *reinterpret_cast<const Vec16<T>*>(srow + c * CH);
                            if (want_dot) {
#pragma unroll
                                for (int e = 0; e < CH; ++e) acc += (double)(y.v[e] * ov[k].v[e]);
                            }
                            if (!tma_dot) stv_stream(P.out + off + (size_t)c * CH, y);
                        }
                    }
                }
            } else if (sizeof(T) == 4 && (n & 1) == 0 && P.vec_ok) {
                for (int c = ln; c < n / 2; c += TW) {
                    const cplx<T> y = *reinterpret_cast<const cplx<T>*>(srow + 2 * c);
                    if (want_dot) {
                        const cplx<T> ov = ld_stream(reinterpret_cast<const cplx<T>*>((const T*)P.v0 + off + 2 * c));
                        acc += (double)(y.x * ov.x) + (double)(y.y * ov.y);
                    }
                    st_stream(reinterpret_cast<cplx<T>*>(P.out + off + 2 * c), y);
                }
            } else {
                for (int i = ln; i < n; i += TW) {
                    const T y = srow[i];
                    if (want_dot) acc += (double)(y * ld_stream((const T*)P.v0 + off + i));
                    st_stream(P.out + off + i, y);
                }
            }
            if (want_dot) {
                acc = team_sum(acc, WPR > 1 ? 32 : tws);
                if (ractive && (WPR > 1 ? l32 == 0 : ln == 0)) s_part[row * WPR + warp % WPR] = acc;
            }
        }
    }
#ifndef HIPGP_EMU
    if (tma_dot && tid == 0) bulk_s2g_wait();
#endif
    if (want_dot) {
        __syncthreads();
        constexpr int WPR2 = (NT / 32) > NROW ? (NT / 32) / NROW : 1;
        if (tid < nl) { double a = 0.0; for (int k = 0; k < WPR2; ++k) a += s_part[tid * WPR2 + k]; P.st.partial[g0 + tid] = a; }
        pcg_finalize(P.st, P.dot_kind, g0, g1, P.nrows, tid, NT);
    }
}

}
```

### hipgp_b200/csrc/plan.cu

```cuda
#include "plan_types.cuh"
#include "setup_kernels.cuh"
#include "kxu_kernels.cuh"

namespace hipgp {
thread_local std::string g_err;
bool g_no_fast = false;
}

namespace hipgp {

template <class T> struct Tag {};
static Geom<float>& geom(hipgp_plan* p, bool wide, Tag<float>) { return wide ? p->gw32 : p->gn32; }
static Geom<double>& geom(hipgp_plan* p, bool wide, Tag<double>) { return wide ? p->gw64 : p->gn64; }

template <class T> static size_t rows_smem(int H, int RBP) { return sizeof(cplx<T>) * (size_t)(H + 1) * RBP; }

template <class T>
static void pick_rows_tiling(long total_rows, int H, int* RB, int* RBP, int* nthreads) {
    int rb = 8;
    while (rb > 1 && (rows_smem<T>(H, rb + 1) > 96 * 1024 || total_rows < (long)rb * 148)) rb >>= 1;
    if (rows_smem<T>(H, rb + 1) > 200 * 1024) throw Error("row axis too long for the shared-memory FFT (L = " + std::to_string(2 * H) + ")");
    *RB = rb; *RBP = rb == 1 ? 1 : rb + 1;
    long work = (long)H * rb / 8;
    *nthreads = work >= 256 ? 256 : (work >= 128 ? 128 : (work >= 64 ? 64 : 32));
}

template <class T> static bool aligned2(const void* p) { return ((uintptr_t)p % (2 * sizeof(T))) == 0; }

template <class T>
static bool launch_rows_fast(hipgp_plan* pl, bool inverse, RowsParams<T>& P, cudaStream_t st) {
    if (g_no_fast) return false;
    switch (P.H) {
#define X(LEN, ...) case LEN: launch_rows_fast_len<T, LEN>(pl, inverse, P, st); return true;
        HIPGP_FAST_LIST(X)
#undef X
        default: return false;
    }
}

template <class T>
static bool geom_allows_fast(const Geom<T>& g) {
    if (sizeof(T) == 8) return true;
    if (g_no_fast || fast_radices(g.H).empty()) return false;
    for (int d = 0; d + 1 < g.D; ++d) if (fast_radices(g.L[d]).empty()) return false;
    return true;
}

template <class T>
static void launch_rows(hipgp_plan* pl, bool inverse, RowsParams<T>& P, cudaStream_t st, bool allow_fast = true) {
    P.vec_ok = (aligned2<T>(P.in) && aligned2<T>(P.out) && aligned2<T>(P.v0) && aligned2<T>(P.v1) && aligned2<T>(P.v2)) ? 1 : 0;
    {
        auto a16 = [](const void* q) { return ((uintptr_t)q % 16) == 0; };
        P.vec16_ok = (a16(P.in) && a16(P.out) && a16(P.v0) && a16(P.v1) && a16(P.v2)) ? 1 : 0;
    }
    if (allow_fast && P.do_fft && launch_rows_fast<T>(pl, inverse, P, st)) return;
    int nth;
    pick_rows_tiling<T>(P.total_rows, P.H, &P.RB, &P.RBP, &nth);
    const size_t smem = rows_smem<T>(P.H, P.RBP);
    dim3 grid((unsigned)((P.total_rows + P.RB - 1) / P.RB));
    PROF_BEGIN(pl, inverse ? 2 : 0, st);
    if (inverse) {
        auto k = rows_inv_kernel<T>;
        if (smem > 48 * 1024) HIPGP_SET_MAX_SMEM(k, smem);
        HIPGP_LAUNCH(k, grid, dim3(nth), smem, st, P);
    } else {
        auto k = rows_fwd_kernel<T>;
        if (smem > 48 * 1024) HIPGP_SET_MAX_SMEM(k, smem);
        HIPGP_LAUNCH(k, grid, dim3(nth), smem, st, P);
    }
    PROF_END(pl, st);
    CK_LAUNCH();
    pl->launches++;
}

template <class T>
static bool launch_cols_fast(hipgp_plan* pl, ColsParams<T>& P, long n_outer, long B, cudaStream_t st) {
    if (g_no_fast) return false;
    switch (P.f.Ln) {
#define X(LEN, ...) case LEN: return launch_cols_fast_len<T, LEN>(pl, P, n_outer, B, st);
        HIPGP_FAST_LIST(X)
#undef X
        default: return false;
    }
}

template <class T>
static void launch_cols(hipgp_plan* pl, ColsParams<T>& P, long n_outer, long B, cudaStream_t st, bool allow_fast = true) {
    if (allow_fast && launch_cols_fast<T>(pl, P, n_outer, B, st)) return;
    const int L = P.f.Ln;
    int tb = sizeof(T) == 4 ? 16 : 8;
    while (tb > 1 && sizeof(cplx<T>) * (size_t)L * (tb + 1) > 100 * 1024) tb >>= 1;
    while (tb > 1 && (long)tb > P.inner) tb >>= 1;
    const int tbp = tb == 1 ? 1 : tb + 1;
    const size_t smem = sizeof(cplx<T>) * (size_t)L * tbp;
    if (smem > 220 * 1024) throw Error("grid axis too long for the shared-memory FFT (L = " + std::to_string(L) + ")");
    P.TB = tb; P.TBP = tbp;
    long work = (long)L * tb / 8;
    int nth = work >= 512 ? 512 : (work >= 256 ? 256 : (work >= 128 ? 128 : (work >= 64 ? 64 : 32)));
    dim3 grid((unsigned)((P.inner + tb - 1) / tb), (unsigned)n_outer, (unsigned)B);
    auto k = cols_pass_kernel<T>;
    if (smem > 48 * 1024) HIPGP_SET_MAX_SMEM(k, smem);
    PROF_BEGIN(pl, 1, st);
    HIPGP_LAUNCH(k, grid, dim3(nth), smem, st, P);
    PROF_END(pl, st);
    CK_LAUNCH();
    pl->launches++;
}

template <class T>
static void rows_geom(RowsParams<T>& R, Geom<T>& g) {
    R.L = g.L[g.D - 1]; R.H = g.H; R.W_pitch = g.P;
    R.f = g.frow.dev; R.twL = g.twL.template as<cplx<T>>(); R.twLp = g.twLp.template as<cplx<T>>();
    R.part = g.part.template as<int>(); R.pairq = g.pairq.template as<int>();
    R.pairs = g.pairs.template as<int>(); R.pairw = g.pairw.template as<cplx<T>>(); R.npair0 = g.npair0;
    R.quadq = g.quadq.template as<int>(); R.quadw = g.quadw.template as<cplx<T>>(); R.nquad = g.nquad;
}

static void ws_elems(int D, const int* L, long P, const int* n_in, const int* n_out, long B, long* w1, long* w2) {
    if (D == 1) { *w1 = B * P; *w2 = 0; return; }
    if (D == 2) { *w1 = B * std::max(n_in[0], n_out[0]) * P; *w2 = 0; return; }
    const long R01 = std::max((long)n_in[0] * n_in[1], (long)n_out[0] * n_out[1]);
    const long R0 = std::max(n_in[0], n_out[0]);
    *w1 = B * R01 * P; *w2 = B * R0 * (long)L[1] * P;
}

template <class T>
static void run_pipeline_group(hipgp_plan* pl, Geom<T>& g, const int* n_in, const int* n_out, const void* spec, int spec_kind,
                         long B, const RowsFusion& ff, const RowsFusion& fi, const PcgDev& st, bool gated, cudaStream_t s) {
    const int D = g.D;
    long w1, w2;
    ws_elems(D, g.L, g.P, n_in, n_out, B, &w1, &w2);
    pl->W1.ensure(sizeof(cplx<T>) * (size_t)w1, &pl->dev_bytes);
    if (w2) pl->W2.ensure(sizeof(cplx<T>) * (size_t)w2, &pl->dev_bytes);
    cplx<T>* W1 = pl->W1.as<cplx<T>>();
    cplx<T>* W2 = pl->W2.as<cplx<T>>();
    const long P = g.P;
    const int* done = gated ? st.flags : nullptr;
    const bool fast = geom_allows_fast(g);

    long rows_in = 1, rows_out = 1;
    for (int d = 0; d + 1 < D; ++d) { rows_in *= n_in[d]; rows_out *= n_out[d]; }
    const long Wrows = std::max(rows_in, rows_out);

    RowsParams<T> R{};
    rows_geom(R, g);
    R.W = W1; R.W_rows = (int)Wrows; R.st = st;
    R.in = (const T*)ff.in; R.v0 = (T*)ff.v0; R.v1 = (T*)ff.v1; R.v2 = (const T*)ff.v2;
    R.mode = ff.mode; R.do_fft = 1; R.total_rows = B * rows_in; R.nrows = (int)rows_in; R.n_real = n_in[D - 1];
    R.spec = nullptr; R.spec_kind = SPEC_NONE;
    launch_rows<T>(pl, false, R, s, fast);

    if (D == 2) {
        ColsParams<T> C{};
        C.in = W1; C.out = W1; C.n_in = n_in[0]; C.n_out = n_out[0]; C.inner = g.H + 1; C.pitch = P;
        C.in_ostride = C.out_ostride = 0; C.in_bstride = C.out_bstride = Wrows * P;
        C.f = g.fcol[0].dev; C.mode = CM_FUSED; C.spec = spec; C.spec_kind = spec_kind; C.done_flag = done;
        launch_cols<T>(pl, C, 1, B, s, fast);
    } else if (D == 3) {
        const long R0 = std::max(n_in[0], n_out[0]);
        const long L1 = g.L[1];
        ColsParams<T> C{};
        C.done_flag = done; C.spec = nullptr; C.spec_kind = SPEC_NONE;
        C.in = W1; C.out = W2; C.n_in = n_in[1]; C.n_out = n_in[1]; C.inner = g.H + 1; C.pitch = P;
        C.in_ostride = (long)n_in[1] * P; C.in_bstride = Wrows * P; C.out_ostride = L1 * P; C.out_bstride = R0 * L1 * P;
        C.f = g.fcol[1].dev; C.mode = CM_FWD;
        launch_cols<T>(pl, C, n_in[0], B, s, fast);
        C.in = W2; C.out = W2; C.n_in = n_in[0]; C.n_out = n_out[0]; C.inner = L1 * P; C.pitch = L1 * P;
        C.in_ostride = C.out_ostride = 0; C.in_bstride = C.out_bstride = R0 * L1 * P;
        C.f = g.fcol[0].dev; C.mode = CM_FUSED; C.spec = spec; C.spec_kind = spec_kind;
        launch_cols<T>(pl, C, 1, B, s, fast);
        C.in = W2; C.out = W1; C.n_in = n_out[1]; C.n_out = n_out[1]; C.inner = g.H + 1; C.pitch = P;
        C.in_ostride = L1 * P; C.in_bstride = R0 * L1 * P; C.out_ostride = (long)n_out[1] * P; C.out_bstride = Wrows * P;
        C.f = g.fcol[1].dev; C.mode = CM_INV; C.spec = nullptr; C.spec_kind = SPEC_NONE;
        launch_cols<T>(pl, C, n_out[0], B, s, fast);
    }

    R.out = (T*)fi.out; R.v0 = (T*)fi.v0; R.mode = fi.mode; R.dot_kind = fi.dot_kind;
    R.total_rows = B * rows_out; R.nrows = (int)rows_out; R.n_real = n_out[D - 1];
    if (D == 1) { R.spec = spec; R.spec_kind = spec_kind; }
    launch_rows<T>(pl, true, R, s, fast);
}


template <class T>
static long pass_group(hipgp_plan* pl, Geom<T>& g, const int* n_in, const int* n_out, long B) {
    static const char* env = getenv("HIPGP_L2_GROUP_MB");
    const double budget_mb = env ? atof(env) : 0.0;
    if (budget_mb <= 0 || B <= 1) return B;
    long w1, w2;
    ws_elems(g.D, g.L, g.P, n_in, n_out, 1, &w1, &w2);
    long vin = 1, vout = 1;
    for (int d = 0; d < g.D; ++d) { vin *= n_in[d]; vout *= n_out[d]; }
    const double per_rhs = (double)sizeof(cplx<T>) * (double)(w1 + w2) + (double)sizeof(T) * (double)(vin + vout);
    long grp = (long)(budget_mb * 1048576.0 / per_rhs);
    (void)pl;
    return std::max<long>(1, std::min<long>(B, grp));
}

template <class T>
static void run_pipeline(hipgp_plan* pl, Geom<T>& g, const int* n_in, const int* n_out, const void* spec, int spec_kind,
                         long B, const RowsFusion& ff, const RowsFusion& fi, const PcgDev& st, bool gated, cudaStream_t s) {
    const long grp = pass_group<T>(pl, g, n_in, n_out, B);
    if (grp >= B) { run_pipeline_group<T>(pl, g, n_in, n_out, spec, spec_kind, B, ff, fi, st, gated, s); return; }
    long vin = 1, vout = 1, rows_in = 1, rows_out = 1;
    for (int d = 0; d < g.D; ++d) { vin *= n_in[d]; vout *= n_out[d]; }
    for (int d = 0; d + 1 < g.D; ++d) { rows_in *= n_in[d]; rows_out *= n_out[d]; }
    auto shift = [](const void* p, long elems) -> const void* { return p ? (const void*)((const T*)p + elems) : nullptr; };
    for (long b0 = 0; b0 < B; b0 += grp) {
        const long nb = std::min(grp, B - b0);
        RowsFusion f2 = ff, i2 = fi;
        f2.in = shift(ff.in, b0 * vin); f2.v0 = (void*)shift(ff.v0, b0 * vin); f2.v1 = (void*)shift(ff.v1, b0 * vin); f2.v2 = shift(ff.v2, b0 * vin);
        i2.out = (void*)shift(fi.out, b0 * vout); i2.v0 = (void*)shift(fi.v0, b0 * vout);
        PcgDev s2 = st;
        if (st.zr) {
            s2.zr = st.zr + b0; s2.zr_prev = st.zr_prev + b0; s2.pAp = st.pAp + b0; s2.rr = st.rr + b0;
            s2.rr_all = st.rr_all ? st.rr_all : st.rr;
            s2.row_cnt = st.row_cnt + b0;
            s2.partial = st.partial + b0 * std::max(rows_in, rows_out);
        }
        run_pipeline_group<T>(pl, g, n_in, n_out, spec, spec_kind, nb, f2, i2, s2, gated, s);
    }
}

static void forward_full(hipgp_plan* pl, Geom<double>& g, const double* h, cudaStream_t s) {
    const int D = g.D;
    long rows = 1;
    for (int d = 0; d + 1 < D; ++d) rows *= g.L[d];
    pl->W1.ensure(sizeof(cplx<double>) * (size_t)rows * g.P, &pl->dev_bytes);
    cplx<double>* W = pl->W1.as<cplx<double>>();
    RowsParams<double> R{};
    rows_geom(R, g);
    R.in = h; R.W = W; R.W_rows = (int)rows; R.mode = RF_PLAIN; R.do_fft = 1;
    R.total_rows = rows; R.nrows = (int)rows; R.n_real = g.L[D - 1];
    launch_rows<double>(pl, false, R, s);
    if (D >= 2) {
        ColsParams<double> C{};
        C.in = W; C.out = W; C.mode = CM_FWD; C.done_flag = nullptr; C.spec_kind = SPEC_NONE;
        if (D == 3) {
            C.n_in = C.n_out = g.L[1]; C.inner = g.H + 1; C.pitch = g.P;
            C.in_ostride = C.out_ostride = (long)g.L[1] * g.P; C.in_bstride = C.out_bstride = 0;
            C.f = g.fcol[1].dev;
            launch_cols<double>(pl, C, g.L[0], 1, s);
            C.n_in = C.n_out = g.L[0]; C.inner = (long)g.L[1] * g.P; C.pitch = (long)g.L[1] * g.P;
            C.in_ostride = C.out_ostride = 0; C.f = g.fcol[0].dev;
            launch_cols<double>(pl, C, 1, 1, s);
        } else {
            C.n_in = C.n_out = g.L[0]; C.inner = g.H + 1; C.pitch = g.P;
            C.in_ostride = C.out_ostride = 0; C.in_bstride = C.out_bstride = 0; C.f = g.fcol[0].dev;
            launch_cols<double>(pl, C, 1, 1, s);
        }
    }
}

static const double* axis_costab(hipgp_plan* pl, int d) {
    DevBuf& b = pl->costabs[d];
    if (!b.p) {
        const int md = pl->m[d];
        const int Nn = md > 1 ? 2 * (md - 1) : 1;
        std::vector<double> tab(Nn);
        for (int t = 0; t < Nn; ++t) tab[t] = md > 1 ? std::cos(M_PI * (double)t / (double)(md - 1)) : 1.0;
        b.ensure(sizeof(double) * Nn, &pl->dev_bytes);
        CK(cudaMemcpy(b.p, tab.data(), sizeof(double) * Nn, cudaMemcpyHostToDevice));
    }
    return b.as<double>();
}

static const double* axis_cosmat(hipgp_plan* pl, int d, cudaStream_t s) {
    const int md = pl->m[d];
    if (md > 2048) return nullptr;
    DevBuf& b = pl->cosmats[d];
    if (!b.p) {
        const double* tab = axis_costab(pl, d);
        const size_t h = (size_t)(md + 1) / 2;
        b.ensure(sizeof(double) * 2 * h * h, &pl->dev_bytes);
        auto k = dct1_cosmat_sym_kernel;
        HIPGP_LAUNCH(k, dim3((unsigned)std::min<size_t>(148 * 4, (2 * h * h + 255) / 256)), dim3(256), 0, s, tab, b.as<double>(), md);
        CK_LAUNCH(); pl->launches++;
    }
    return b.as<double>();
}

static void dct_all_axes(hipgp_plan* pl, const double* in, double* out, double* tmp, bool normalise, cudaStream_t s) {
    const double* src = in;
    const int D = pl->D;
    double* bufs[2] = {out, tmp};
    int which = (D % 2 == 1) ? 0 : 1;
    static const char* env_old = getenv("HIPGP_DCT_DENSE");
    for (int d = 0; d < D; ++d) {
        const int md = pl->m[d];
        long inner = 1, outer = 1;
        for (int e = d + 1; e < D; ++e) inner *= pl->m[e];
        for (int e = 0; e < d; ++e) outer *= pl->m[e];
        const double* tab = axis_costab(pl, d);
        const int Nn = md > 1 ? 2 * (md - 1) : 1;
        double* dst = bufs[which];
        const double scale = normalise ? 1.0 / (double)Nn : 1.0;
        if (env_old) {
            int bx = 64;
            while (bx > 1 && bx / 2 >= inner) bx >>= 1;
            dim3 block(bx, 256 / bx);
            const int nx = (int)((inner + bx - 1) / bx);
            dim3 grid((unsigned)((long)nx * outer), (unsigned)((md + block.y - 1) / block.y), 1);
            auto k = dct1_axis_kernel;
            HIPGP_LAUNCH(k, grid, block, 0, s, src, dst, tab, md, inner, scale, nx);
        } else if (inner == 1) {
            dim3 grid((unsigned)((md + 63) / 64), (unsigned)((outer + 127) / 128), 1);
            const double* cw = md > 2 ? axis_cosmat(pl, d, s) : nullptr;
            if (cw) {
                const int hk0 = (md + 1) / 2;
                dim3 gs((unsigned)((hk0 + 63) / 64), (unsigned)((outer + 127) / 128), 2);
                auto k = dct1_sym_kernel<true>; HIPGP_LAUNCH(k, gs, dim3(256), 0, s, src, dst, cw, md, inner, outer, scale, 0);
            } else { auto k = dct1_tile_kernel<true>; HIPGP_LAUNCH(k, grid, dim3(256), 0, s, src, dst, tab, md, inner, outer, scale); }
        } else {
            if (outer > 65535) throw Error("DCT set-up: more than 65535 outer slices");
            dim3 grid((unsigned)((inner + 63) / 64), (unsigned)((md + 127) / 128), (unsigned)outer);
            const double* cw = md > 2 ? axis_cosmat(pl, d, s) : nullptr;
            if (cw) {
                const int hk0 = (md + 1) / 2, nty = (hk0 + 127) / 128;
                dim3 gs((unsigned)((inner + 63) / 64), (unsigned)(2 * nty), (unsigned)outer);
                auto k = dct1_sym_kernel<false>; HIPGP_LAUNCH(k, gs, dim3(256), 0, s, src, dst, cw, md, inner, outer, scale, nty);
            } else { auto k = dct1_tile_kernel<false>; HIPGP_LAUNCH(k, grid, dim3(256), 0, s, src, dst, tab, md, inner, outer, scale); }
        }
        CK_LAUNCH();
        pl->launches++;
        src = dst; which ^= 1;
    }
}

template <class T>
static void build_spectrum(hipgp_plan* pl, bool wide, const double* col, DevBuf& dst, bool complex_spec, cudaStream_t s) {
    Geom<double>& g = wide ? pl->gw64 : pl->gn64;
    EmbedDims e{};
    e.D = g.D;
    long total = 1;
    for (int d = 0; d < 3; ++d) { e.m[d] = 1; e.N[d] = 1; e.L[d] = 1; e.wide[d] = 0; }
    for (int d = 0; d < g.D; ++d) {
        const int slot = 3 - g.D + d;
        e.m[slot] = pl->m[d]; e.N[slot] = pl->N[d]; e.L[slot] = g.L[d]; e.wide[slot] = wide ? (pl->wide_real ? 2 : 1) : 0;
        total *= g.L[d];
    }
    pl->tmpB.ensure(sizeof(double) * (size_t)total, &pl->dev_bytes);
    {
        auto k = embed_kernel;
        const int nb = (int)std::min<long>((total + 255) / 256, 148 * 8);
        HIPGP_LAUNCH(k, dim3(nb), dim3(256), 0, s, col, pl->tmpB.as<double>(), e);
        CK_LAUNCH(); pl->launches++;
    }
    forward_full(pl, g, pl->tmpB.as<double>(), s);
    const long n = g.spec_elems();
    double scale = 0.25;
    for (int d = 0; d < g.D; ++d) scale /= (double)g.L[d];
    const unsigned nblk = (unsigned)((n + 255) / 256);
    if (complex_spec) {
        dst.ensure(sizeof(cplx<T>) * (size_t)n, &pl->dev_bytes);
        auto k = store_spec_cplx_kernel<T>; HIPGP_LAUNCH(k, dim3(nblk), dim3(256), 0, s, pl->W1.as<cplx<double>>(), dst.as<cplx<T>>(), n, scale);
    } else {
        dst.ensure(sizeof(T) * (size_t)n, &pl->dev_bytes);
        auto k = store_spec_real_kernel<T>; HIPGP_LAUNCH(k, dim3(nblk), dim3(256), 0, s, pl->W1.as<cplx<double>>(), dst.as<T>(), n, scale);
    }
    CK_LAUNCH(); pl->launches++;
}

template <class T>
static void ensure_geoms(hipgp_plan* pl, bool wide) {
    Geom<double>& g64 = wide ? pl->gw64 : pl->gn64;
    const int* L = wide ? pl->Lw : pl->Ln;
    if (!g64.built) g64.build(pl->D, L, &pl->dev_bytes);
    if (sizeof(T) == 4) {
        Geom<float>& g32 = wide ? pl->gw32 : pl->gn32;
        if (!g32.built) g32.build(pl->D, L, &pl->dev_bytes);
    }
}

template <class T>
static void set_first_row(hipgp_plan* pl, const void* column, double clampv, cudaStream_t s) {
    const long M = pl->M;
    pl->clampv = clampv;
    ensure_geoms<T>(pl, false);
    for (DevBuf* b : {&pl->Dm, &pl->Dinv, &pl->Dsqrt, &pl->colK, &pl->colG, &pl->colS, &pl->tmpA})
        b->ensure(sizeof(double) * (size_t)M, &pl->dev_bytes);
    pl->tmpB.ensure(sizeof(double) * (size_t)M, &pl->dev_bytes);
    pl->counts.ensure(sizeof(unsigned) * 4, &pl->dev_bytes);
    CK(cudaMemsetAsync(pl->counts.p, 0, sizeof(unsigned) * 4, s));
    const unsigned nb = (unsigned)((M + 255) / 256);
    {
        auto k = to_double_kernel<T>;
        HIPGP_LAUNCH(k, dim3(nb), dim3(256), 0, s, (const T*)column, pl->colK.as<double>(), M);
        CK_LAUNCH(); pl->launches++;
    }
    dct_all_axes(pl, pl->colK.as<double>(), pl->tmpA.as<double>(), pl->tmpB.as<double>(), false, s);
    {
        auto k = clamp_derive_kernel<T>;
        HIPGP_LAUNCH(k, dim3(nb), dim3(256), 0, s, pl->tmpA.as<double>(), pl->Dm.as<double>(), pl->Dinv.as<double>(),
                     pl->Dsqrt.as<double>(), M, clampv, pl->counts.as<unsigned>());
        CK_LAUNCH(); pl->launches++;
    }
    unsigned hc[4] = {0, 0, 0, 0};
    CK(cudaMemcpyAsync(hc, pl->counts.p, sizeof(hc), cudaMemcpyDeviceToHost, s));
    CK(cudaStreamSynchronize(s));
    pl->nclamped = hc[0];
    if (pl->nclamped != 0 || sizeof(T) == 4)
        dct_all_axes(pl, pl->Dm.as<double>(), pl->colK.as<double>(), pl->tmpB.as<double>(), true, s);
    dct_all_axes(pl, pl->Dinv.as<double>(), pl->colG.as<double>(), pl->tmpB.as<double>(), true, s);
    build_spectrum<T>(pl, false, pl->colK.as<double>(), pl->specK, false, s);
    build_spectrum<T>(pl, false, pl->colG.as<double>(), pl->specCinv, false, s);
    pl->have_spec = true; pl->have_wide = false; pl->have_slabK = pl->have_slabCinv = false;
}

template <class T>
static void ensure_wide(hipgp_plan* pl, cudaStream_t s) {
    if (pl->have_wide) return;
    ensure_geoms<T>(pl, true);
    static const char* env_c = getenv("HIPGP_WIDE_COMPLEX");
    bool real_ok = !env_c;
    for (int d = 0; d < pl->D; ++d) if (pl->Lw[d] < 2 * pl->N[d] - 1) real_ok = false;
    pl->wide_real = real_ok;
    dct_all_axes(pl, pl->Dsqrt.as<double>(), pl->colS.as<double>(), pl->tmpB.as<double>(), true, s);
    build_spectrum<T>(pl, true, pl->colS.as<double>(), pl->specW, !real_ok, s);
    pl->have_wide = true;
}

static PcgDev null_state() { PcgDev st{}; return st; }

template <class T>
static void matvec(hipgp_plan* pl, int mode, const void* in, void* out, long B, cudaStream_t s) {
    if (!pl->have_spec) throw Error("plan has no spectrum: call hipgp_plan_set_first_row first");
    if (B < 0) throw Error("negative number of right-hand sides");
    if (B == 0) return;
    if (!in || !out) throw Error("null vector pointer");
    RowsFusion ff, fi;
    ff.mode = RF_PLAIN; ff.in = in; fi.mode = RI_PLAIN; fi.out = out;
    const bool wide = (mode == HIPGP_MV_RT || mode == HIPGP_MV_R);
    if (wide) ensure_wide<T>(pl, s);
    Geom<T>& g = geom(pl, wide, Tag<T>());
    int n_in[3], n_out[3];
    for (int d = 0; d < pl->D; ++d) {
        n_in[d] = mode == HIPGP_MV_R ? pl->N[d] : pl->m[d];
        n_out[d] = mode == HIPGP_MV_RT ? pl->N[d] : pl->m[d];
    }
    const void* spec; int kind;
    switch (mode) {
        case HIPGP_MV_K: spec = pl->specK.p; kind = SPEC_REAL; break;
        case HIPGP_MV_CINV: spec = pl->specCinv.p; kind = SPEC_REAL; break;
        case HIPGP_MV_RT: spec = pl->specW.p; kind = pl->wide_real ? SPEC_REAL : SPEC_CPLX; break;
        case HIPGP_MV_R: spec = pl->specW.p; kind = pl->wide_real ? SPEC_REAL : SPEC_CPLX_CONJ; break;
        default: throw Error("unknown matvec mode");
    }
    run_pipeline<T>(pl, g, n_in, n_out, spec, kind, B, ff, fi, null_state(), false, s);
}

template <class T>
static PcgDev pcg_state(hipgp_plan* pl, long B, double tol, bool cg_mode) {
    const long M = pl->M;
    long nrows = 1;
    for (int d = 0; d + 1 < pl->D; ++d) nrows *= pl->m[d];
    for (DevBuf* b : {&pl->vr, &pl->vp, &pl->vz, &pl->vAp}) b->ensure(sizeof(T) * (size_t)(B * M), &pl->dev_bytes);
    pl->partial.ensure(sizeof(double) * (size_t)(B * nrows), &pl->dev_bytes);
    pl->scal.ensure(sizeof(double) * (size_t)(4 * B), &pl->dev_bytes);
    const bool fresh = pl->cnt.bytes < sizeof(unsigned) * (size_t)(B + 1);
    pl->cnt.ensure(sizeof(unsigned) * (size_t)(B + 1), &pl->dev_bytes);
    pl->flags.ensure(sizeof(int) * 4, &pl->dev_bytes);
    if (fresh) CK(cudaMemset(pl->cnt.p, 0, pl->cnt.bytes));
    PcgDev st{};
    double* sc = pl->scal.as<double>();
    st.zr = sc; st.zr_prev = sc + B; st.pAp = sc + 2 * B; st.rr = sc + 3 * B;
    st.partial = pl->partial.as<double>();
    st.row_cnt = pl->cnt.as<unsigned>(); st.rhs_cnt = pl->cnt.as<unsigned>() + B;
    st.flags = pl->flags.as<int>();
    st.tol = tol; st.B = (int)B; st.cg_mode = cg_mode ? 1 : 0;
    return st;
}

template <class T>
static void launch_vec(hipgp_plan* pl, int mode, const PcgDev& st, long B, const void* in, void* v0, void* v1, const void* v2,
                       cudaStream_t s) {
    long nrows = 1;
    for (int d = 0; d + 1 < pl->D; ++d) nrows *= pl->m[d];
    RowsParams<T> R{};
    R.in = (const T*)in; R.v0 = (T*)v0; R.v1 = (T*)v1; R.v2 = (const T*)v2;
    R.mode = mode; R.do_fft = 0; R.total_rows = B * nrows; R.nrows = (int)nrows; R.n_real = pl->m[pl->D - 1];
    R.H = (R.n_real + 1) / 2; R.L = 2 * R.H; R.st = st;
    R.RB = 8; R.RBP = 9;
    dim3 grid((unsigned)((R.total_rows + R.RB - 1) / R.RB));
    auto k = rows_fwd_kernel<T>;
    PROF_BEGIN(pl, 3, s);
    HIPGP_LAUNCH(k, grid, dim3(256), 0, s, R);
    PROF_END(pl, s);
    CK_LAUNCH(); pl->launches++;
}

template <class T>
static void pcg_begin(hipgp_plan* pl, const void* b, void* x, long B, double tol, bool precond, cudaStream_t s) {
    if (!pl->have_spec) throw Error("plan has no spectrum: call hipgp_plan_set_first_row first");
    if (B <= 0) throw Error("pcg needs at least one right-hand side");
    if (!b || !x) throw Error("null vector pointer");
    const long M = pl->M;
    PcgDev st = pcg_state<T>(pl, B, tol, !precond);
    if (!pl->pinned) CK(cudaMallocHost(&pl->pinned, 64));
    Geom<T>& g = geom(pl, false, Tag<T>());
    int nn[3];
    for (int d = 0; d < pl->D; ++d) nn[d] = pl->m[d];
    T* r = pl->vr.as<T>(); T* z = precond ? pl->vz.as<T>() : r;
    CK(cudaMemsetAsync(x, 0, sizeof(T) * (size_t)(B * M), s));
    CK(cudaMemcpyAsync(r, b, sizeof(T) * (size_t)(B * M), cudaMemcpyDeviceToDevice, s));
    CK(cudaMemsetAsync(st.flags, 0, sizeof(int) * 4, s));
    CK(cudaMemsetAsync(reinterpret_cast<char*>(st.flags) + 2 * sizeof(int), 1, 1, s));
    RowsFusion ff, fi;
    if (precond) {
        ff.mode = RF_PLAIN; ff.in = r; fi.mode = RI_DOT; fi.dot_kind = DOT_ZR; fi.out = z; fi.v0 = r;
        run_pipeline<T>(pl, g, nn, nn, pl->specCinv.p, SPEC_REAL, B, ff, fi, st, false, s);
    } else {
        launch_vec<T>(pl, RF_SELFDOT, st, B, r, nullptr, nullptr, nullptr, s);
    }
    pl->run_x = x; pl->run_B = B; pl->run_precond = precond; pl->run_tol = tol; pl->run_active = true;
}

template <class T>
static void pcg_iterate(hipgp_plan* pl, int niter, cudaStream_t s) {
    if (!pl->run_active) throw Error("hipgp_pcg_step without hipgp_pcg_begin");
    const long B = pl->run_B;
    const bool precond = pl->run_precond;
    PcgDev st = pcg_state<T>(pl, B, pl->run_tol, !precond);
    Geom<T>& g = geom(pl, false, Tag<T>());
    int nn[3];
    for (int d = 0; d < pl->D; ++d) nn[d] = pl->m[d];
    T* r = pl->vr.as<T>(); T* p = pl->vp.as<T>(); T* z = precond ? pl->vz.as<T>() : r; T* Ap = pl->vAp.as<T>();
    void* x = pl->run_x;
    RowsFusion ff, fi;
    for (int c = 0; c < niter; ++c) {
        ff = RowsFusion(); fi = RowsFusion();
        ff.mode = RF_PUPDATE; ff.in = z; ff.v0 = p;
        fi.mode = RI_DOT; fi.dot_kind = DOT_PAP; fi.out = Ap; fi.v0 = p;
        run_pipeline<T>(pl, g, nn, nn, pl->specK.p, SPEC_REAL, B, ff, fi, st, true, s);
        if (precond) {
            ff = RowsFusion(); fi = RowsFusion();
            ff.mode = RF_XRUPDATE; ff.in = Ap; ff.v0 = r; ff.v1 = x; ff.v2 = p;
            fi.mode = RI_DOT; fi.dot_kind = DOT_ZR; fi.out = z; fi.v0 = r;
            run_pipeline<T>(pl, g, nn, nn, pl->specCinv.p, SPEC_REAL, B, ff, fi, st, true, s);
        } else {
            launch_vec<T>(pl, RF_XRUPDATE, st, B, Ap, r, x, p, s);
        }
    }
}

static void pcg_poll(hipgp_plan* pl, int* done, int* iters, double* max_resid, double* resid_out, cudaStream_t s) {
    int* hflags = reinterpret_cast<int*>(pl->pinned);
    CK(cudaMemcpyAsync(hflags, pl->flags.p, sizeof(int) * 4, cudaMemcpyDeviceToHost, s));
    std::vector<double> rr;
    if (max_resid || resid_out) {
        rr.resize(pl->run_B);
        CK(cudaMemcpyAsync(rr.data(), pl->scal.as<double>() + 3 * pl->run_B, sizeof(double) * pl->run_B, cudaMemcpyDeviceToHost, s));
    }
    CK(cudaStreamSynchronize(s));
    if (done) *done = hflags[0];
    if (iters) *iters = hflags[1];
    if (max_resid) {
        double mx = 0.0; bool nan = false;
        for (double v : rr) { const double q = std::sqrt(v); if (q != q) nan = true; else if (q > mx) mx = q; }
        *max_resid = nan ? NAN : mx;
    }
    if (resid_out) for (long i = 0; i < pl->run_B; ++i) resid_out[i] = std::sqrt(rr[i]);
}

template <class T>
static void pcg(hipgp_plan* pl, const void* b, void* x, long B, int maxiter, double tol, bool precond, int* iters_out,
                int* callbacks_out, double* resid_out, hipgp_iter_cb cb, void* user, cudaStream_t s) {
    if (iters_out) *iters_out = 0;
    if (callbacks_out) *callbacks_out = 0;
    if (B < 0) throw Error("negative number of right-hand sides");
    if (B == 0) return;
    pcg_begin<T>(pl, b, x, B, tol, precond, s);
    const int check_every = cb ? 1 : 8;
    int done = 0, iters = 0, n = 0;
    while (n < maxiter && !done) {
        const int chunk = std::min(check_every, maxiter - n);
        pcg_iterate<T>(pl, chunk, s);
        pcg_poll(pl, &done, &iters, nullptr, nullptr, s);
        n += chunk;
        if (cb && !done) cb(n - 1, x, user);
    }
    if (iters_out) *iters_out = iters;
    if (callbacks_out) *callbacks_out = done ? iters - 1 : iters;
    if (resid_out) pcg_poll(pl, nullptr, nullptr, nullptr, resid_out, s);
    pl->run_active = false;
}

}

#define API_BEGIN try {
#define API_END                                                                          \
    } catch (const std::exception& e) { hipgp::g_err = e.what(); return -1; }            \
      catch (...) { hipgp::g_err = "unknown error"; return -2; }                         \
    return 0;

#define DISPATCH(pl, call_f32, call_f64) do { if ((pl)->dtype == HIPGP_F32) { call_f32; } else { call_f64; } } while (0)

static void need_plan(const hipgp_plan* pl) { if (!pl) throw Error("null plan handle"); }
static void set_device(const hipgp_plan* pl) { need_plan(pl); CK(cudaSetDevice(pl->device)); }

static void slab_peer_close(hipgp_plan* pl) {
#ifndef HIPGP_EMU
    for (int i = 0; i < pl->n_ipc_opened; ++i) if (pl->ipc_opened[i]) cudaIpcCloseMemHandle(pl->ipc_opened[i]);
#endif
    pl->n_ipc_opened = 0; pl->peers_ready = false;
}

extern "C" {

const char* hipgp_last_error(void) { return hipgp::g_err.c_str(); }
int hipgp_version(void) { return 100; }

int hipgp_plan_create(int ndim, const int64_t* m, int dtype, int device, hipgp_plan** out) {
    API_BEGIN
    if (!out || !m || ndim < 1) throw Error("bad arguments");
    if (dtype != HIPGP_F32 && dtype != HIPGP_F64) throw Error("dtype must be HIPGP_F32 or HIPGP_F64");
    hipgp_plan* pl = new hipgp_plan();
    pl->dtype = dtype; pl->device = device; pl->ndim_user = ndim;
    int D = 0;
    for (int d = 0; d < ndim; ++d) {
        if (m[d] < 1) { delete pl; throw Error("grid extents must be >= 1"); }
        pl->m_user.push_back((long)m[d]);
        pl->M *= m[d];
        if (m[d] > 1) {
            if (D == 3) { delete pl; throw Error("at most 3 grid axes of extent > 1 are supported"); }
            pl->m[D] = (int)m[d]; pl->N[D] = 2 * (int)m[d] - 2; pl->E *= pl->N[D]; ++D;
        }
    }
    if (D == 0) { D = 1; pl->m[0] = 1; pl->N[0] = 1; }
    pl->D = D;
    const char* nf = getenv("HIPGP_NO_FAST");
    g_no_fast = nf && nf[0] == '1';
    const char* env = getenv("HIPGP_POW2_ONLY");
    const bool pow2 = env && env[0] == '1';
    for (int d = 0; d < D; ++d) {
        const bool row = (d == D - 1);
        pl->Ln[d] = choose_length(2L * pl->m[d] - 1, row, pow2);
        pl->Lw[d] = choose_length((long)pl->N[d] + pl->m[d] - 1, row, pow2);
    }
    *out = pl;
    API_END
}

int hipgp_plan_destroy(hipgp_plan* pl) {
    API_BEGIN
    if (!pl) return 0;
    size_t* t = &pl->dev_bytes;
    pl->gn32.release(t); pl->gw32.release(t); pl->gn64.release(t); pl->gw64.release(t);
    for (DevBuf* b : {&pl->specK, &pl->specCinv, &pl->specW, &pl->Dm, &pl->Dinv, &pl->Dsqrt, &pl->colK, &pl->colG, &pl->colS,
                      &pl->tmpA, &pl->tmpB, &pl->costab, &pl->counts, &pl->W1, &pl->W2, &pl->vr, &pl->vp, &pl->vz, &pl->vAp,
                      &pl->partial, &pl->scal, &pl->cnt, &pl->flags, &pl->stage_in, &pl->stage_out, &pl->corrU, &pl->corrV, &pl->corrS,
                      &pl->corrLag, &pl->gradA, &pl->slabSpecK, &pl->slabSpecCinv, &pl->slabR1, &pl->slabR2, &pl->slot_in[0], &pl->slot_in[1], &pl->slot_out[0], &pl->slot_out[1], &pl->costabs[0], &pl->costabs[1], &pl->costabs[2], &pl->cosmats[0], &pl->cosmats[1], &pl->cosmats[2]})
        b->release(t);
    slab_peer_close(pl);
#ifndef HIPGP_EMU
    for (auto& se : pl->slot_ev) for (auto& e : se) if (e) cudaEventDestroy(e);
    if (pl->slot_flags) cudaFreeHost(pl->slot_flags);
#else
    delete[] pl->slot_flags;
#endif
    if (pl->pinned) cudaFreeHost(pl->pinned);
#ifndef HIPGP_EMU
    for (auto& cs : pl->copy_streams) if (cs) cudaStreamDestroy(cs);
#endif
    delete pl;
    API_END
}

int hipgp_plan_sizes(const hipgp_plan* pl, int64_t* M, int64_t* Mprime) {
    API_BEGIN
    need_plan(pl);
    if (M) *M = pl->M;
    if (Mprime) *Mprime = pl->E;
    API_END
}

int hipgp_plan_embedding(const hipgp_plan* pl, int64_t* Ln, int64_t* Lw) {
    API_BEGIN
    need_plan(pl);
    int a = 0;
    for (int d = 0; d < pl->ndim_user; ++d) {
        const bool active = pl->m_user[d] > 1 || (pl->D == 1 && pl->M == 1 && d == 0);
        if (Ln) Ln[d] = active ? pl->Ln[a] : 1;
        if (Lw) Lw[d] = active ? pl->Lw[a] : 1;
        if (active) ++a;
    }
    API_END
}

int hipgp_plan_set_first_row(hipgp_plan* pl, const void* column, double clampv, int64_t* clamped_out, void* stream) {
    API_BEGIN
    set_device(pl);
    DISPATCH(pl, set_first_row<float>(pl, column, clampv, (cudaStream_t)stream), set_first_row<double>(pl, column, clampv, (cudaStream_t)stream));
    if (clamped_out) *clamped_out = pl->nclamped;
    API_END
}

int hipgp_plan_spectrum(hipgp_plan* pl, int which, void* out, void* stream) {
    API_BEGIN
    set_device(pl);
    if (!pl->have_spec) throw Error("plan has no spectrum");
    if (which < 0 || which > 3) throw Error("bad spectrum selector");
    EmbedDims e{};
    for (int d = 0; d < 3; ++d) { e.m[d] = 1; e.N[d] = 1; e.L[d] = 1; e.wide[d] = 0; }
    for (int d = 0; d < pl->D; ++d) { const int slot = 3 - pl->D + d; e.m[slot] = pl->m[d]; e.N[slot] = pl->N[d]; }
    const int nb = (int)std::min<long>((pl->E + 255) / 256, 148 * 8);
    cudaStream_t s = (cudaStream_t)stream;
    if (pl->dtype == HIPGP_F32) { auto k = expand_even_kernel<float>; HIPGP_LAUNCH(k, dim3(nb), dim3(256), 0, s, pl->Dm.as<double>(), (float*)out, e, which); }
    else { auto k = expand_even_kernel<double>; HIPGP_LAUNCH(k, dim3(nb), dim3(256), 0, s, pl->Dm.as<double>(), (double*)out, e, which); }
    CK_LAUNCH(); pl->launches++;
    API_END
}

int hipgp_matvec(hipgp_plan* pl, int mode, const void* in, void* out, int64_t B, void* stream) {
    API_BEGIN
    set_device(pl);
    DISPATCH(pl, matvec<float>(pl, mode, in, out, (long)B, (cudaStream_t)stream), matvec<double>(pl, mode, in, out, (long)B, (cudaStream_t)stream));
    API_END
}

static size_t elem_size(const hipgp_plan* pl) { return pl->dtype == HIPGP_F32 ? 4 : 8; }

int hipgp_matvec_host(hipgp_plan* pl, int mode, const void* in_host, void* out_host, int64_t B, void* stream) {
    API_BEGIN
    set_device(pl);
    cudaStream_t s = (cudaStream_t)stream;
    const size_t nin = (size_t)B * (mode == HIPGP_MV_R ? pl->E : pl->M) * elem_size(pl);
    const size_t nout = (size_t)B * (mode == HIPGP_MV_RT ? pl->E : pl->M) * elem_size(pl);
    pl->stage_in.ensure(nin, &pl->dev_bytes); pl->stage_out.ensure(nout, &pl->dev_bytes);
    CK(cudaMemcpyAsync(pl->stage_in.p, in_host, nin, cudaMemcpyHostToDevice, s));
    DISPATCH(pl, matvec<float>(pl, mode, pl->stage_in.p, pl->stage_out.p, (long)B, s), matvec<double>(pl, mode, pl->stage_in.p, pl->stage_out.p, (long)B, s));
    CK(cudaMemcpyAsync(out_host, pl->stage_out.p, nout, cudaMemcpyDeviceToHost, s));
    CK(cudaStreamSynchronize(s));
    API_END
}

int hipgp_pcg(hipgp_plan* pl, const void* b, void* x, int64_t B, int maxiter, double tol, int precond, int* iters_out,
              int* callbacks_out, double* resid_out, hipgp_iter_cb cb, void* user, void* stream) {
    API_BEGIN
    set_device(pl);
    cudaStream_t s = (cudaStream_t)stream;
    DISPATCH(pl, pcg<float>(pl, b, x, (long)B, maxiter, tol, precond != 0, iters_out, callbacks_out, resid_out, cb, user, s),
             pcg<double>(pl, b, x, (long)B, maxiter, tol, precond != 0, iters_out, callbacks_out, resid_out, cb, user, s));
    API_END
}

int hipgp_pcg_begin(hipgp_plan* pl, const void* b, void* x, int64_t B, double tol, int precond, void* stream) {
    API_BEGIN
    set_device(pl);
    cudaStream_t s = (cudaStream_t)stream;
    DISPATCH(pl, pcg_begin<float>(pl, b, x, (long)B, tol, precond != 0, s), pcg_begin<double>(pl, b, x, (long)B, tol, precond != 0, s));
    API_END
}

int hipgp_pcg_step(hipgp_plan* pl, int niter, int* done_out, int* iters_out, double* max_resid_out, void* stream) {
    API_BEGIN
    set_device(pl);
    cudaStream_t s = (cudaStream_t)stream;
    DISPATCH(pl, pcg_iterate<float>(pl, niter, s), pcg_iterate<double>(pl, niter, s));
    if (done_out || iters_out || max_resid_out) pcg_poll(pl, done_out, iters_out, max_resid_out, nullptr, s);
    API_END
}

int hipgp_pcg_host(hipgp_plan* pl, const void* b_host, void* x_host, int64_t B, int maxiter, double tol, int precond,
                   int* iters_out, int* callbacks_out, double* resid_out, void* stream) {
    API_BEGIN
    set_device(pl);
    cudaStream_t s = (cudaStream_t)stream;
    const size_t n = (size_t)B * pl->M * elem_size(pl);
    pl->stage_in.ensure(n, &pl->dev_bytes); pl->stage_out.ensure(n, &pl->dev_bytes);
    CK(cudaMemcpyAsync(pl->stage_in.p, b_host, n, cudaMemcpyHostToDevice, s));
    DISPATCH(pl, pcg<float>(pl, pl->stage_in.p, pl->stage_out.p, (long)B, maxiter, tol, precond != 0, iters_out, callbacks_out, resid_out, nullptr, nullptr, s),
             pcg<double>(pl, pl->stage_in.p, pl->stage_out.p, (long)B, maxiter, tol, precond != 0, iters_out, callbacks_out, resid_out, nullptr, nullptr, s));
    CK(cudaMemcpyAsync(x_host, pl->stage_out.p, n, cudaMemcpyDeviceToHost, s));
    CK(cudaStreamSynchronize(s));
    API_END
}

int hipgp_pcg_host_pipelined(hipgp_plan* pl, const void* b_host, void* x_host, int64_t B, int maxiter, double tol, int precond,
                             int64_t group, int* iters_out, void* stream) {
    API_BEGIN
    set_device(pl);
    if (iters_out) *iters_out = 0;
    if (B < 0) throw Error("negative number of right-hand sides");
    if (B == 0) return 0;
    if (!b_host || !x_host) throw Error("null vector pointer");
    if (group <= 0 || group > B) group = B;
    cudaStream_t s = (cudaStream_t)stream;
#ifndef HIPGP_EMU
    if (!pl->copy_streams[0]) {
        CK(cudaStreamCreateWithFlags(&pl->copy_streams[0], cudaStreamNonBlocking));
        CK(cudaStreamCreateWithFlags(&pl->copy_streams[1], cudaStreamNonBlocking));
    }
#endif
    const size_t row = (size_t)pl->M * elem_size(pl);
    pl->stage_in.ensure((size_t)B * row, &pl->dev_bytes); pl->stage_out.ensure((size_t)B * row, &pl->dev_bytes);
    std::vector<long> gs;
    if (B >= 4 * group) { gs.push_back(group); gs.push_back(B - 2 * group); gs.push_back(group); }
    else for (long b0 = 0; b0 < B; b0 += group) gs.push_back(std::min<long>(group, B - b0));
    const long ng = (long)gs.size();
    std::vector<long> gb0(ng);
    { long acc = 0; for (long g = 0; g < ng; ++g) { gb0[g] = acc; acc += gs[g]; } }
    std::vector<cudaEvent_t> in_ready(ng), solved(ng);
#ifndef HIPGP_EMU
    for (long g = 0; g < ng; ++g) { CK(cudaEventCreateWithFlags(&in_ready[g], cudaEventDisableTiming)); CK(cudaEventCreateWithFlags(&solved[g], cudaEventDisableTiming)); }
    cudaStream_t cin = pl->copy_streams[0], cout = pl->copy_streams[1];
    cudaEvent_t start; CK(cudaEventCreateWithFlags(&start, cudaEventDisableTiming));
    CK(cudaEventRecord(start, s)); CK(cudaStreamWaitEvent(cin, start, 0)); CK(cudaStreamWaitEvent(cout, start, 0));
#else
    cudaStream_t cin = s, cout = s;
#endif
    for (long g = 0; g < ng; ++g) {
        const long b0 = gb0[g], nb = gs[g];
        CK(cudaMemcpyAsync((char*)pl->stage_in.p + b0 * row, (const char*)b_host + b0 * row, nb * row, cudaMemcpyHostToDevice, cin));
#ifndef HIPGP_EMU
        CK(cudaEventRecord(in_ready[g], cin));
#endif
    }
    int iters_max = 0;
    for (long g = 0; g < ng; ++g) {
        const long b0 = gb0[g], nb = gs[g];
#ifndef HIPGP_EMU
        CK(cudaStreamWaitEvent(s, in_ready[g], 0));
#endif
        int it = 0;
        void* bg = (char*)pl->stage_in.p + b0 * row; void* xg = (char*)pl->stage_out.p + b0 * row;
        DISPATCH(pl, pcg<float>(pl, bg, xg, nb, maxiter, tol, precond != 0, &it, nullptr, nullptr, nullptr, nullptr, s),
                 pcg<double>(pl, bg, xg, nb, maxiter, tol, precond != 0, &it, nullptr, nullptr, nullptr, nullptr, s));
        iters_max = std::max(iters_max, it);
#ifndef HIPGP_EMU
        CK(cudaEventRecord(solved[g], s));
        CK(cudaStreamWaitEvent(cout, solved[g], 0));
#endif
        CK(cudaMemcpyAsync((char*)x_host + b0 * row, xg, nb * row, cudaMemcpyDeviceToHost, cout));
    }
#ifndef HIPGP_EMU
    CK(cudaStreamSynchronize(cout));
    CK(cudaStreamSynchronize(s));
    for (long g = 0; g < ng; ++g) { cudaEventDestroy(in_ready[g]); cudaEventDestroy(solved[g]); }
    cudaEventDestroy(start);
#endif
    if (iters_out) *iters_out = iters_max;
    API_END
}

int hipgp_pcg_host_submit(hipgp_plan* pl, const void* b_host, void* x_host, int64_t B, int maxiter, double tol, int precond, int slot,
                          void* stream) {
    API_BEGIN
    set_device(pl);
    if (slot < 0 || slot > 1) throw Error("slot must be 0 or 1");
    if (B <= 0) throw Error("hipgp_pcg_host_submit needs at least one right-hand side");
    if (!b_host || !x_host) throw Error("null vector pointer");
    if (maxiter < 0) throw Error("negative maxiter");
    cudaStream_t s = (cudaStream_t)stream;
#ifndef HIPGP_EMU
    if (!pl->copy_streams[0]) {
        CK(cudaStreamCreateWithFlags(&pl->copy_streams[0], cudaStreamNonBlocking));
        CK(cudaStreamCreateWithFlags(&pl->copy_streams[1], cudaStreamNonBlocking));
    }
    for (int e = 0; e < 3; ++e) if (!pl->slot_ev[slot][e]) CK(cudaEventCreateWithFlags(&pl->slot_ev[slot][e], cudaEventDisableTiming));
    if (!pl->slot_flags) CK(cudaMallocHost((void**)&pl->slot_flags, sizeof(int) * 8));
    if (pl->slot_busy[slot]) { CK(cudaEventSynchronize(pl->slot_ev[slot][2])); pl->slot_busy[slot] = false; }
    cudaStream_t cin = pl->copy_streams[0], cout = pl->copy_streams[1];
#else
    if (!pl->slot_flags) pl->slot_flags = new int[8];
    cudaStream_t cin = s, cout = s;
#endif
    const size_t n = (size_t)B * pl->M * elem_size(pl);
    pl->slot_in[slot].ensure(n, &pl->dev_bytes); pl->slot_out[slot].ensure(n, &pl->dev_bytes);
    CK(cudaMemcpyAsync(pl->slot_in[slot].p, b_host, n, cudaMemcpyHostToDevice, cin));
#ifndef HIPGP_EMU
    CK(cudaEventRecord(pl->slot_ev[slot][0], cin));
    CK(cudaStreamWaitEvent(s, pl->slot_ev[slot][0], 0));
#endif
    if (pl->dtype == HIPGP_F32) { pcg_begin<float>(pl, pl->slot_in[slot].p, pl->slot_out[slot].p, (long)B, tol, precond != 0, s); pcg_iterate<float>(pl, maxiter, s); }
    else { pcg_begin<double>(pl, pl->slot_in[slot].p, pl->slot_out[slot].p, (long)B, tol, precond != 0, s); pcg_iterate<double>(pl, maxiter, s); }
    pl->run_active = false;
    CK(cudaMemcpyAsync(pl->slot_flags + 4 * slot, pl->flags.p, sizeof(int) * 4, cudaMemcpyDeviceToHost, s));
#ifndef HIPGP_EMU
    CK(cudaEventRecord(pl->slot_ev[slot][1], s));
    CK(cudaStreamWaitEvent(cout, pl->slot_ev[slot][1], 0));
#endif
    CK(cudaMemcpyAsync(x_host, pl->slot_out[slot].p, n, cudaMemcpyDeviceToHost, cout));
#ifndef HIPGP_EMU
    CK(cudaEventRecord(pl->slot_ev[slot][2], cout));
#endif
    pl->slot_busy[slot] = true;
    API_END
}
int hipgp_pcg_host_wait(hipgp_plan* pl, int slot, int* iters_out) {
    API_BEGIN
    set_device(pl);
    if (slot < 0 || slot > 1) throw Error("slot must be 0 or 1");
    if (!pl->slot_busy[slot]) throw Error("hipgp_pcg_host_wait: nothing was submitted on this slot");
#ifndef HIPGP_EMU
    CK(cudaEventSynchronize(pl->slot_ev[slot][2]));
#endif
    pl->slot_busy[slot] = false;
    if (iters_out) *iters_out = pl->slot_flags[4 * slot + 1];
    API_END
}

int hipgp_compute_kn(hipgp_plan* pl, const void* Knm, void* kn, int64_t B, int maxiter, double tol, int* iters_out, void* stream) {
    API_BEGIN
    set_device(pl);
    cudaStream_t s = (cudaStream_t)stream;
    const size_t n = (size_t)B * pl->M * elem_size(pl);
    pl->stage_out.ensure(n, &pl->dev_bytes);
    void* d0 = pl->stage_out.p;
    DISPATCH(pl, pcg<float>(pl, Knm, d0, (long)B, maxiter, tol, true, iters_out, nullptr, nullptr, nullptr, nullptr, s),
             pcg<double>(pl, Knm, d0, (long)B, maxiter, tol, true, iters_out, nullptr, nullptr, nullptr, nullptr, s));
    DISPATCH(pl, matvec<float>(pl, HIPGP_MV_RT, d0, kn, (long)B, s), matvec<double>(pl, HIPGP_MV_RT, d0, kn, (long)B, s));
    API_END
}

int hipgp_plan_profile(hipgp_plan* pl, int enable) {
    API_BEGIN
    need_plan(pl);
    pl->profiling = enable != 0;
    API_END
}
int hipgp_plan_profile_read(hipgp_plan* pl, int kernel_class, double* ms_total, int64_t* launches, int reset) {
    API_BEGIN
    need_plan(pl);
    if (kernel_class < 0 || kernel_class > 3) throw Error("kernel_class must be 0..3");
#ifndef HIPGP_EMU
    set_device(pl);
    CK(cudaDeviceSynchronize());
    for (auto& r : pl->prof) {
        float ms = 0;
        CK(cudaEventElapsedTime(&ms, r.e0, r.e1));
        pl->prof_ms[r.cls] += ms; pl->prof_n[r.cls] += 1;
        cudaEventDestroy(r.e0); cudaEventDestroy(r.e1);
    }
    pl->prof.clear();
#endif
    if (ms_total) *ms_total = pl->prof_ms[kernel_class];
    if (launches) *launches = pl->prof_n[kernel_class];
    if (reset) for (int i = 0; i < 4; ++i) { pl->prof_ms[i] = 0; pl->prof_n[i] = 0; }
    API_END
}
int hipgp_plan_device_bytes(const hipgp_plan* pl, size_t* bytes) { API_BEGIN need_plan(pl); if (bytes) *bytes = pl->dev_bytes; API_END }
int hipgp_plan_launch_count(const hipgp_plan* pl, int64_t* launches) { API_BEGIN need_plan(pl); if (launches) *launches = pl->launches; API_END }

}

#include "vec_api.inl"
#include "kxu_api.inl"
#include "corr_api.inl"
#include "block_api.inl"
#include "slab_api.inl"

#ifdef HIPGP_EMU
namespace emu {
thread_local dim3 t_threadIdx, t_blockIdx;
dim3 g_blockDim, g_gridDim;
Barrier g_block_barrier;
Barrier g_warp_barrier[64];
NamedBarrier g_named_barrier[16];
unsigned char* g_dyn_smem = nullptr;
double g_shfl_scratch[64][32][2];
}
#endif
```

### hipgp_b200/csrc/plan_types.cuh

```cuda
#pragma once
#include "../../include/hipgp_b200.h"
#include "conv_kernels.cuh"

#include <string>
#include <stdexcept>

namespace hipgp {

extern thread_local std::string g_err;
struct Error : std::runtime_error { using std::runtime_error::runtime_error; };

#define CK(expr)                                                                                     \
    do {                                                                                             \
        cudaError_t e__ = (expr);                                                                    \
        if (e__ != cudaSuccess)                                                                      \
            throw Error(std::string(#expr) + ": " + cudaGetErrorString(e__));                        \
    } while (0)
#define CK_LAUNCH() CK(cudaGetLastError())

struct DevBuf {
    void* p = nullptr; size_t bytes = 0;
    void ensure(size_t n, size_t* total) {
        if (n <= bytes) return;
        if (p) { cudaFree(p); *total -= bytes; }
        p = nullptr; bytes = 0;
        if (cudaMalloc(&p, n) != cudaSuccess) { p = nullptr; throw Error("cudaMalloc of " + std::to_string(n) + " bytes failed"); }
        bytes = n; *total += n;
    }
    void release(size_t* total) { if (p) { cudaFree(p); *total -= bytes; } p = nullptr; bytes = 0; }
    template <class U> U* as() const { return reinterpret_cast<U*>(p); }
};

#ifdef HIPGP_DEV_SMALL
#if defined(HIPGP_EXP) && HIPGP_EXP == 1
#define HIPGP_EXP_R2048 8, 8, 8, 4
#define HIPGP_EXP_R1024 8, 8, 4, 4
#elif defined(HIPGP_EXP) && HIPGP_EXP == 2
#define HIPGP_EXP_R2048 8, 16, 16
#define HIPGP_EXP_R1024 8, 8, 16
#else
#define HIPGP_EXP_R2048 16, 8, 16
#define HIPGP_EXP_R1024 8, 8, 16
#endif
#define HIPGP_FAST_LIST_G0(X) X(2048, HIPGP_EXP_R2048)
#define HIPGP_FAST_LIST_G1(X) X(16, 16)
#define HIPGP_FAST_LIST_G2(X) X(1024, HIPGP_EXP_R1024) X(128, 8, 16)
#define HIPGP_FAST_LIST_G3(X) X(64, 4, 16) X(32, 8, 4)
#define HIPGP_FAST_LIST_G4(X)
#else
#define HIPGP_FAST_LIST_G0(X) X(2048, 16, 8, 16) X(8192, 16, 8, 8, 8)
#define HIPGP_FAST_LIST_G1(X) X(4096, 16, 16, 16) X(16, 16) X(8, 8) X(4, 4)
#define HIPGP_FAST_LIST_G2(X) X(1024, 8, 8, 16) X(512, 4, 8, 16) X(256, 16, 16) X(128, 8, 16)
#define HIPGP_FAST_LIST_G3(X) X(3072, 3, 16, 8, 8) X(1536, 3, 8, 8, 8) X(768, 3, 16, 16) X(64, 4, 16) X(32, 8, 4)
#define HIPGP_FAST_LIST_G4(X) X(640, 5, 8, 16) X(320, 5, 4, 16) X(384, 3, 8, 16) X(192, 3, 4, 16) X(96, 3, 8, 4)
#endif
#define HIPGP_FAST_LIST(X) HIPGP_FAST_LIST_G0(X) HIPGP_FAST_LIST_G1(X) HIPGP_FAST_LIST_G2(X) HIPGP_FAST_LIST_G3(X) HIPGP_FAST_LIST_G4(X)

extern bool g_no_fast;

inline std::vector<int> fast_radices(int Ln) {
    switch (Ln) {
#define X(LEN, ...) case LEN: return std::vector<int>{__VA_ARGS__};
        HIPGP_FAST_LIST(X)
#undef X
        default: return {};
    }
}

inline std::vector<int> choose_radices(int Ln) {
    std::vector<int> r = fast_radices(Ln);
    if (!r.empty()) return r;
    int n = Ln;
    while (n % 5 == 0) { r.push_back(5); n /= 5; }
    while (n % 3 == 0) { r.push_back(3); n /= 3; }
    int e = 0;
    while (n % 2 == 0) { ++e; n /= 2; }
    if (n != 1) throw Error("FFT length " + std::to_string(Ln) + " is not 2^a 3^b 5^c");
    while (e >= 4) { r.push_back(16); e -= 4; }
    if (e == 3) r.push_back(8); else if (e == 2) r.push_back(4); else if (e == 1) r.push_back(2);
    return r;
}

inline double fft_cost(int Ln) {
    std::vector<int> r = choose_radices(Ln);
    double c = 0;
    for (int x : r) c += (x == 3 || x == 5) ? 1.3 : 1.0;
    const bool fast = !fast_radices(Ln).empty();
    return (double)Ln * (c + 0.5) * (fast ? 1.0 : 2.5);
}

inline bool is_smooth(long n) {
    for (int p : {2, 3, 5}) while (n % p == 0) n /= p;
    return n == 1;
}

inline int choose_length(long n, bool even, bool pow2_only) {
    if (n < 2) n = 2;
    long best = -1; double bc = 0;
    for (long L = n; L <= 2 * n + 2; ++L) {
        if (even && (L & 1)) continue;
        if (pow2_only ? ((L & (L - 1)) != 0) : !is_smooth(L)) continue;
        const double c = even ? 2.0 * fft_cost((int)(L / 2)) : fft_cost((int)L);
        if (best < 0 || c < bc) { best = L; bc = c; }
    }
    if (best < 0) throw Error("no embedding length found");
    return (int)best;
}

template <class T>
struct LineFftHost {
    LineFft<T> dev{};
    DevBuf tw, rev, pos, twst;
    std::vector<int> hrev_, hpos_;
    void build(int Ln, size_t* total) {
        std::vector<int> r = Ln > 1 ? choose_radices(Ln) : std::vector<int>();
        if ((int)r.size() > kMaxStages) throw Error("too many FFT stages");
        dev.Ln = Ln; dev.nst = (int)r.size();
        for (size_t i = 0; i < r.size(); ++i) dev.radix[i] = r[i];
        std::vector<cplx<T>> htw(Ln);
        for (int k = 0; k < Ln; ++k) {
            const double a = -2.0 * M_PI * (double)k / (double)Ln;
            htw[k].x = (T)std::cos(a); htw[k].y = (T)std::sin(a);
        }
        std::vector<int> hrev(Ln), hpos(Ln);
        for (int k = 0; k < Ln; ++k) {
            int kk = k, p = 0, span = Ln;
            for (size_t i = 0; i < r.size(); ++i) { span /= r[i]; p += (kk % r[i]) * span; kk /= r[i]; }
            hpos[k] = p; hrev[p] = k;
        }
        tw.ensure(sizeof(cplx<T>) * Ln, total); rev.ensure(sizeof(int) * Ln, total); pos.ensure(sizeof(int) * Ln, total);
        CK(cudaMemcpy(tw.p, htw.data(), sizeof(cplx<T>) * Ln, cudaMemcpyHostToDevice));
        CK(cudaMemcpy(rev.p, hrev.data(), sizeof(int) * Ln, cudaMemcpyHostToDevice));
        CK(cudaMemcpy(pos.p, hpos.data(), sizeof(int) * Ln, cudaMemcpyHostToDevice));
        dev.tw = tw.as<cplx<T>>(); dev.rev = rev.as<int>(); dev.pos = pos.as<int>();
        hrev_ = hrev; hpos_ = hpos;
        std::vector<cplx<T>> st;
        int Nt = Ln;
        auto tw_entry = [](int j, int rr, int Nt_) {
            const long num = ((long)j * rr) % Nt_;
            const double a = -2.0 * M_PI * (double)num / (double)Nt_;
            cplx<T> wv; wv.x = (T)std::cos(a); wv.y = (T)std::sin(a);
            return wv;
        };
        for (size_t i = 0; i < r.size(); ++i) {
            const int R = r[i], S = Nt / R;
            dev.twoff[i] = (int)st.size();
            if (TwLayout<T>::paired) {
                for (int p = 0; p < R / 2; ++p)
                    for (int j = 0; j < S; ++j)
                        for (int e = 0; e < 2; ++e) {
                            const int rr = 2 * p + 1 + e;
                            cplx<T> one; one.x = (T)1; one.y = (T)0;
                            st.push_back(rr < R ? tw_entry(j, rr, Nt) : one);
                        }
            } else {
                for (int rr = 1; rr < R; ++rr)
                    for (int j = 0; j < S; ++j) st.push_back(tw_entry(j, rr, Nt));
            }
            Nt = S;
        }
        if (st.empty()) st.resize(1);
        twst.ensure(sizeof(cplx<T>) * st.size(), total);
        CK(cudaMemcpy(twst.p, st.data(), sizeof(cplx<T>) * st.size(), cudaMemcpyHostToDevice));
        dev.twst = twst.as<cplx<T>>();
    }
    void release(size_t* total) { tw.release(total); rev.release(total); pos.release(total); twst.release(total); }
};

template <class T>
struct Geom {
    int D = 0;
    int L[3] = {1, 1, 1};
    int H = 1;
    long P = 0;
    LineFftHost<T> fcol[2];
    LineFftHost<T> frow;
    DevBuf twL, twLp, part, pairq, pairs, pairw, quadq, quadw;
    int npair0 = 0, nquad = 0;
    bool built = false;
    void build(int D_, const int* L_, size_t* total) {
        D = D_;
        for (int d = 0; d < D; ++d) L[d] = L_[d];
        H = L[D - 1] / 2;
        P = ((long)H + 1 + 7) / 8 * 8;
        for (int d = 0; d + 1 < D; ++d) fcol[d].build(L[d], total);
        frow.build(H, total);
        std::vector<cplx<T>> w(H);
        for (int k = 0; k < H; ++k) {
            const double a = -2.0 * M_PI * (double)k / (double)L[D - 1];
            w[k].x = (T)std::cos(a); w[k].y = (T)std::sin(a);
        }
        twL.ensure(sizeof(cplx<T>) * H, total);
        CK(cudaMemcpy(twL.p, w.data(), sizeof(cplx<T>) * H, cudaMemcpyHostToDevice));
        std::vector<cplx<T>> wp(H); std::vector<int> pt(H);
        for (int q = 0; q < H; ++q) {
            const int k = frow.hrev_[q];
            wp[q] = w[k];
            pt[q] = k == 0 ? 0 : frow.hpos_[H - k];
        }
        std::vector<int> pq;
        for (int q = 0; q < H; ++q) if (q <= pt[q]) pq.push_back(q);
        if ((int)pq.size() != H / 2 + 1) throw Error("internal: r2c pair table has the wrong size");
        pairq.ensure(sizeof(int) * pq.size(), total);
        CK(cudaMemcpy(pairq.p, pq.data(), sizeof(int) * pq.size(), cudaMemcpyHostToDevice));
        {
            const std::vector<int> rad = H > 1 ? choose_radices(H) : std::vector<int>();
            const int RL = rad.empty() ? 1 : rad.back();
            bool ok = rad.size() > 1 && RL % 2 == 0 && H % 2 == 0;
            std::vector<int> qd; std::vector<cplx<T>> qw;
            for (int qa = RL; ok && qa < H; qa += 2) {
                const int pa = pt[qa], pa1 = pt[qa + 1];
                if (pa != pa1 + 1 || (pa1 & 1) || pa1 < RL) { ok = false; break; }
                if (qa <= pa1) { qd.push_back(qa); qd.push_back(pa1); qw.push_back(wp[qa]); qw.push_back(wp[qa + 1]); }
            }
            if (!ok) { qd.clear(); qw.clear(); }
            nquad = (int)(qd.size() / 2);
            npair0 = 0;
            if (ok) { for (int q : pq) if (q < RL) ++npair0; } else npair0 = (int)pq.size();
            if (npair0 + 2 * nquad - (ok ? 0 : 0) < 0) throw Error("internal: quad table");
            std::vector<int> pr; std::vector<cplx<T>> pw;
            for (int q : pq) { pr.push_back(q); pr.push_back(q == 0 ? H : pt[q]); pw.push_back(wp[q]); }
            pairs.ensure(sizeof(int) * pr.size(), total); pairw.ensure(sizeof(cplx<T>) * pw.size(), total);
            CK(cudaMemcpy(pairs.p, pr.data(), sizeof(int) * pr.size(), cudaMemcpyHostToDevice));
            CK(cudaMemcpy(pairw.p, pw.data(), sizeof(cplx<T>) * pw.size(), cudaMemcpyHostToDevice));
            quadq.ensure(sizeof(int) * std::max<size_t>(qd.size(), 2), total); quadw.ensure(sizeof(cplx<T>) * std::max<size_t>(qw.size(), 2), total);
            if (!qd.empty()) {
                CK(cudaMemcpy(quadq.p, qd.data(), sizeof(int) * qd.size(), cudaMemcpyHostToDevice));
                CK(cudaMemcpy(quadw.p, qw.data(), sizeof(cplx<T>) * qw.size(), cudaMemcpyHostToDevice));
            }
        }
        twLp.ensure(sizeof(cplx<T>) * H, total); part.ensure(sizeof(int) * H, total);
        CK(cudaMemcpy(twLp.p, wp.data(), sizeof(cplx<T>) * H, cudaMemcpyHostToDevice));
        CK(cudaMemcpy(part.p, pt.data(), sizeof(int) * H, cudaMemcpyHostToDevice));
        built = true;
    }
    long spec_elems() const { long n = P; for (int d = 0; d + 1 < D; ++d) n *= L[d]; return n; }
    void release(size_t* total) { for (auto& f : fcol) f.release(total); frow.release(total); twL.release(total); twLp.release(total); part.release(total); pairq.release(total); pairs.release(total); pairw.release(total); quadq.release(total); quadw.release(total); built = false; }
};

struct RowsFusion {
    int mode = 0, dot_kind = 0, do_fft = 1;
    const void* in = nullptr; void* out = nullptr; void* v0 = nullptr; void* v1 = nullptr; const void* v2 = nullptr;
};

}

using namespace hipgp;

struct hipgp_plan {
    int dtype = 0, device = 0;
    int ndim_user = 0;
    std::vector<long> m_user;
    int D = 0;
    int m[3] = {1, 1, 1}, N[3] = {1, 1, 1};
    long M = 1, E = 1;
    int Ln[3] = {1, 1, 1}, Lw[3] = {1, 1, 1};
    size_t dev_bytes = 0;
    long launches = 0;
    bool have_spec = false, have_wide = false;
    bool wide_real = false;
    double clampv = 1e-6;
    long nclamped = 0;

    Geom<float> gn32, gw32;
    Geom<double> gn64, gw64;
    DevBuf specK, specCinv, specW;
    DevBuf Dm, Dinv, Dsqrt, colK, colG, colS, tmpA, tmpB, costab, counts;
    DevBuf W1, W2;
    DevBuf vr, vp, vz, vAp, partial, scal, cnt, flags;
    DevBuf stage_in, stage_out;
    DevBuf slabSpecK, slabSpecCinv;
    bool have_slabK = false, have_slabCinv = false;
    DevBuf costabs[3], cosmats[3];
    DevBuf gradA;
    DevBuf corrU, corrV, corrS, corrLag;
    void* pinned = nullptr;
    cudaStream_t copy_streams[2] = {nullptr, nullptr};
    DevBuf slot_in[2], slot_out[2];
    cudaEvent_t slot_ev[2][3] = {{nullptr, nullptr, nullptr}, {nullptr, nullptr, nullptr}};
    bool slot_busy[2] = {false, false};
    int* slot_flags = nullptr;
    long pcg_B = 0;
    DevBuf slabR1, slabR2;
    void* peerR1[16] = {}; void* peerR2[16] = {};
    void* ipc_opened[32] = {}; int n_ipc_opened = 0;
    bool peers_ready = false;
    int slab_chunks = 1;
    int slab_rank = 0, slab_nranks = 1;
    void* run_x = nullptr; long run_B = 0; bool run_precond = true; double run_tol = 0; bool run_active = false;
    bool profiling = false;
    struct ProfRec { int cls; cudaEvent_t e0, e1; };
    std::vector<ProfRec> prof;
    double prof_ms[4] = {0, 0, 0, 0};
    long prof_n[4] = {0, 0, 0, 0};
};

#ifdef HIPGP_EMU
#define PROF_BEGIN(pl, cls, st) ((void)0)
#define PROF_END(pl, st) ((void)0)
#else
#define PROF_BEGIN(pl, cls_, st)                                                   \
    if ((pl)->profiling) {                                                         \
        hipgp_plan::ProfRec r__; r__.cls = (cls_);                                 \
        cudaEventCreate(&r__.e0); cudaEventCreate(&r__.e1);                        \
        cudaEventRecord(r__.e0, (st)); (pl)->prof.push_back(r__);                  \
    }
#define PROF_END(pl, st) if ((pl)->profiling) cudaEventRecord((pl)->prof.back().e1, (st));
#endif


namespace hipgp {
template <class T, int LEN> void launch_rows_fast_len(hipgp_plan* pl, bool inverse, RowsParams<T>& P, cudaStream_t st);
template <class T, int LEN> bool launch_cols_fast_len(hipgp_plan* pl, ColsParams<T>& P, long n_outer, long B, cudaStream_t st);
}
```

Baseline: 451.5.

## Compute PCG dot products in spectral domain inside fused column kernel via Parseval

For 2D/3D grids, the PCG dot products (pAp, zr) are now accumulated during the spectral multiply in the fused column kernels, using Parseval-weighted sums of spec*|v|^2 with half-weights at the DC and Nyquist columns. Per-tile partials are published to global memory and the last tile per batch reduces them. This lets the final rows kernel run in plain mode instead of dot mode, cutting a read of v0 and the dot reduction from that pass. It adds double-precision accumulation, atomics and a partial buffer sized by spectral lines, and it relies on the spectrum being real and the Hermitian weighting being exact.

```diff
diff --git a/hipgp_b200/csrc/cols_blk_kernel.cuh b/hipgp_b200/csrc/cols_blk_kernel.cuh
--- a/hipgp_b200/csrc/cols_blk_kernel.cuh
+++ b/hipgp_b200/csrc/cols_blk_kernel.cuh
@@ -106,6 +106,8 @@
     }
 
     const int mode = P.mode;
+    const bool dot = mode == CM_FUSED && P.dot;
+    __shared__ double s_dot[NT / 32];
     const size_t pitch = (size_t)P.pitch;
     const size_t spitch = P.spec_pitch ? (size_t)P.spec_pitch : (size_t)P.pitch;
     const long ntiles = (long)P.nx * P.ny * P.nz;
@@ -265,6 +267,7 @@
         }
         {
             constexpr int NIT = Cfg::IB3 / GS;
+            double dsum = 0.0;
 #pragma unroll
             for (int k = 0; k < NIT; ++k) {
                 const int q = u + k * GS;
@@ -282,7 +285,19 @@
                     for (int r = 0; r < RLAST; ++r) v[r] = base[r * NL];
                     lbfly<RLAST, false, T>(v);
                 }
-                if (mode == CM_FUSED) {
+                if (dot) {
+                    typename LaneAcc<T>::type acc{};
+                    if (spec_smem) {
+                        const unsigned char* sp = side + ((size_t)sslot(p0) * NL + lane) * SPEC_LANE;
+#pragma unroll
+                        for (int r = 0; r < RLAST; ++r) v[r] = lane_spec_dot(v[r], lane_real_ld((const T*)nullptr, sp + r * NL * SPEC_LANE), acc);
+                    } else if (ok) {
+                        const size_t sidx = (size_t)p0 * spitch + c0 + lane * LPT;
+#pragma unroll
+                        for (int r = 0; r < RLAST; ++r) v[r] = lane_spec_dot(v[r], lane_real_ldg(reinterpret_cast<const T*>(P.spec), sidx + (size_t)r * spitch), acc);
+                    }
+                    dsum += lane_dot_total(P, c0 + lane * LPT, acc);
+                } else if (mode == CM_FUSED) {
                     if (spec_smem) {
                         const unsigned char* sp = side + ((size_t)sslot(p0) * NL + lane) * SPEC_LANE;
 #pragma unroll
@@ -305,6 +320,7 @@
                     for (int r = 0; r < RLAST; ++r) base[r * NL] = v[r];
                 }
             }
+            if (dot) spec_dot_warp(dsum, s_dot, tid);
         }
         if (mode == CM_FWD) continue;
         const bool early_in = tma_in && mode == CM_FUSED && spec_smem;
@@ -339,6 +355,12 @@
         }
         __syncthreads();
         if (mode == CM_FUSED && spec_smem && !early_in) stage_next(t + gridDim.x);
+        unsigned dot_done = 0;
+        if (dot && tid < 32) {
+            int b, ti;
+            spec_dot_tile(P, t, b, ti);
+            dot_done = spec_dot_publish(P.st, s_dot, NT / 32, (long)b * P.nx * P.ny + ti, b, tid);
+        }
         {
 #pragma unroll 1
             for (int it = tid; it < S0 * NL; it += NT) {
@@ -366,6 +388,11 @@
                 }
             }
         }
+        if (dot && tid < 32) {
+            int b, ti;
+            spec_dot_tile(P, t, b, ti);
+            spec_dot_finish(P.st, P.dot - 1, dot_done, b, P.nx * P.ny, tid);
+        }
     }
 }
 
diff --git a/hipgp_b200/csrc/conv_kernels.cuh b/hipgp_b200/csrc/conv_kernels.cuh
--- a/hipgp_b200/csrc/conv_kernels.cuh
+++ b/hipgp_b200/csrc/conv_kernels.cuh
@@ -225,7 +225,7 @@
     cplx<T>* s = reinterpret_cast<cplx<T>*>(smem_raw);
     const int tid = threadIdx.x, nthreads = blockDim.x;
     const int warp = tid >> 5, lane = tid & 31, nwarps = nthreads >> 5;
-    if (P.mode != RI_PLAIN && P.st.flags[0]) return;
+    if (P.st.flags && P.st.flags[0]) return;
     const long g0 = (long)blockIdx.x * P.RB;
     const long g1 = g0 + P.RB < P.total_rows ? g0 + P.RB : P.total_rows;
     const int nl = (int)(g1 - g0);
@@ -307,11 +307,60 @@
     int tma_spec;
     int batch_fastest;
     const int* done_flag;
+    int dot;
+    long dot_P; int dot_H;
+    PcgDev st;
     int out_split_len; long out_split_stride;
     int in_split_len; long in_split_stride;
 };
 template <class T> __device__ __forceinline__ size_t cols_rowoff(int i, long pitch, int split_len, long split_stride) {
     return split_len ? (size_t)(i / split_len) * split_stride + (size_t)(i % split_len) * pitch : (size_t)i * pitch;
+}
+
+template <class T> __device__ __forceinline__ double spec_dot_weight(const ColsParams<T>& P, long c) {
+    if (c >= P.inner) return 0.0;
+    const unsigned q = P.inner <= P.dot_P ? (unsigned)c : (unsigned)c % (unsigned)P.dot_P, H = (unsigned)P.dot_H;
+    return (q == 0 || q == H) ? 0.5 : (q < H ? 1.0 : 0.0);
+}
+template <class T> __device__ __forceinline__ double spec_dot_line(const ColsParams<T>& P, long c, double acc) {
+    const double w = spec_dot_weight(P, c);
+    return w != 0.0 ? w * acc : 0.0;
+}
+
+template <class T> __device__ __forceinline__ void spec_dot_tile(const ColsParams<T>& P, long t, int& b, int& ti) {
+    long bx, by, bz;
+    if (P.batch_fastest) { bz = t % P.nz; const long r = t / P.nz; bx = r % P.nx; by = r / P.nx; }
+    else { bx = t % P.nx; const long r = t / P.nx; by = r % P.ny; bz = r / P.ny; }
+    b = (int)bz; ti = (int)(by * P.nx + bx);
+}
+__device__ __forceinline__ void spec_dot_warp(double acc, double* s_warp, int tid) {
+    acc = warp_sum(acc);
+    if ((tid & 31) == 0) s_warp[tid >> 5] = acc;
+}
+__device__ __forceinline__ unsigned spec_dot_publish(const PcgDev& st, const double* s_warp, int nw, long slot, int b, int lane) {
+    unsigned done = 0;
+    if (lane == 0) {
+        double a = 0.0;
+        for (int w = 0; w < nw; ++w) a += s_warp[w];
+        st.partial[slot] = a;
+        __threadfence();
+        done = atomicAdd(st.row_cnt + b, 1u) + 1u;
+    }
+    return done;
+}
+__device__ __forceinline__ void spec_dot_finish(const PcgDev& st, int kind, unsigned done, int b, int ntile, int lane) {
+    if (__shfl_sync(0xffffffffu, done, 0) != (unsigned)ntile) return;
+    __threadfence();
+    const volatile double* part = st.partial + (long)b * ntile;
+    double acc = 0.0;
+    for (int i = lane; i < ntile; i += 32) acc += part[i];
+    acc = warp_sum(acc);
+    if (lane == 0) {
+        st.row_cnt[b] = 0;
+        if (kind == DOT_PAP) st.pAp[b] = acc;
+        else { st.zr_prev[b] = st.zr[b]; st.zr[b] = acc; }
+        __threadfence();
+    }
 }
 
 template <class T>
@@ -336,11 +385,22 @@
     __syncthreads();
 
     if (P.mode != CM_INV) fft_forward(s, TBP, TB, P.f, tid, nthreads);
+    __shared__ double s_warp[16];
     if (P.mode == CM_FUSED) {
+        double acc = 0.0;
         for (int w = tid; w < L * TB; w += nthreads) {
             const int c = w % TB, i = w / TB;
-            if (c < nc) s[(size_t)i * TBP + c] = apply_spec(s[(size_t)i * TBP + c], P.spec, P.spec_kind, (size_t)i * (P.spec_pitch ? P.spec_pitch : P.pitch) + c0 + c);
-        }
+            if (c < nc) {
+                const size_t sidx = (size_t)i * (P.spec_pitch ? P.spec_pitch : P.pitch) + c0 + c;
+                const cplx<T> v = s[(size_t)i * TBP + c];
+                if (P.dot) {
+                    const double wt = spec_dot_weight(P, c0 + c);
+                    if (wt != 0.0) acc += wt * (double)reinterpret_cast<const T*>(P.spec)[sidx] * ((double)v.x * v.x + (double)v.y * v.y);
+                }
+                s[(size_t)i * TBP + c] = apply_spec(v, P.spec, P.spec_kind, sidx);
+            }
+        }
+        if (P.dot) spec_dot_warp(acc, s_warp, tid);
         __syncthreads();
     }
     if (P.mode != CM_FWD) fft_inverse(s, TBP, TB, P.f, tid, nthreads);
@@ -350,7 +410,12 @@
         const int c = w % TB, i = w / TB;
         if (c < nc) out[cols_rowoff<T>(i, P.pitch, P.out_split_len, P.out_split_stride) + c] = s[(size_t)i * TBP + c];
     }
-}
-
-
-}
+    if (P.mode == CM_FUSED && P.dot && tid < 32) {
+        const int ntile = (int)(gridDim.x * gridDim.y), b = (int)blockIdx.z;
+        const unsigned done = spec_dot_publish(P.st, s_warp, nthreads >> 5, (long)b * ntile + blockIdx.y * gridDim.x + blockIdx.x, b, tid);
+        spec_dot_finish(P.st, P.dot - 1, done, b, ntile, tid);
+    }
+}
+
+
+}
diff --git a/hipgp_b200/csrc/cuda_emu.h b/hipgp_b200/csrc/cuda_emu.h
--- a/hipgp_b200/csrc/cuda_emu.h
+++ b/hipgp_b200/csrc/cuda_emu.h
@@ -146,6 +146,17 @@
     emu::g_warp_barrier[w].wait();
     return r;
 }
+template <class T>
+static inline T __shfl_sync(unsigned, T v, int src) {
+    const int tid = (int)(threadIdx.x + blockDim.x * (threadIdx.y + blockDim.y * threadIdx.z));
+    const int w = tid >> 5, l = tid & 31;
+    std::memcpy(emu::g_shfl_scratch[w][l], &v, sizeof(T));
+    emu::g_warp_barrier[w].wait();
+    T r;
+    std::memcpy(&r, emu::g_shfl_scratch[w][src & 31], sizeof(T));
+    emu::g_warp_barrier[w].wait();
+    return r;
+}
 static inline unsigned atomicAdd(unsigned* p, unsigned v) { return __atomic_fetch_add(p, v, __ATOMIC_SEQ_CST); }
 static inline int atomicAdd(int* p, int v) { return __atomic_fetch_add(p, v, __ATOMIC_SEQ_CST); }
 static inline unsigned atomicInc_emu(unsigned* p) { return __atomic_fetch_add(p, 1u, __ATOMIC_SEQ_CST); }
diff --git a/hipgp_b200/csrc/fast_kernels.cuh b/hipgp_b200/csrc/fast_kernels.cuh
--- a/hipgp_b200/csrc/fast_kernels.cuh
+++ b/hipgp_b200/csrc/fast_kernels.cuh
@@ -36,6 +36,26 @@
     Lane<float> r; r.re = __fmul2_rn(v.re, s2); r.im = __fmul2_rn(v.im, s2); return r;
 }
 __device__ __forceinline__ Lane<double> lane_spec_smem(Lane<double> v, const void* p) { return lscale(v, *reinterpret_cast<const double*>(p)); }
+
+template <class T> struct LaneAcc;
+template <> struct LaneAcc<float> { using type = float2; };
+template <> struct LaneAcc<double> { using type = double; };
+__device__ __forceinline__ Lane<float> lane_spec_dot(Lane<float> v, float2 s, float2& acc) {
+    acc = __ffma2_rn(__ffma2_rn(v.re, v.re, __fmul2_rn(v.im, v.im)), s, acc);
+    Lane<float> r; r.re = __fmul2_rn(v.re, s); r.im = __fmul2_rn(v.im, s); return r;
+}
+__device__ __forceinline__ Lane<double> lane_spec_dot(Lane<double> v, double s, double& acc) {
+    acc += s * (v.re * v.re + v.im * v.im);
+    return lscale(v, s);
+}
+__device__ __forceinline__ float2 lane_real_ld(const float*, const void* p) { return *reinterpret_cast<const float2*>(p); }
+__device__ __forceinline__ double lane_real_ld(const double*, const void* p) { return *reinterpret_cast<const double*>(p); }
+__device__ __forceinline__ float2 lane_real_ldg(const float* spec, size_t idx) { const cplx<float> s = ld_stream(reinterpret_cast<const cplx<float>*>(spec + idx)); return make_float2(s.x, s.y); }
+__device__ __forceinline__ double lane_real_ldg(const double* spec, size_t idx) { return ld_stream(spec + idx); }
+__device__ __forceinline__ double lane_dot_total(const ColsParams<float>& P, long c, float2 acc) {
+    return spec_dot_line(P, c, (double)acc.x) + spec_dot_line(P, c + 1, (double)acc.y);
+}
+__device__ __forceinline__ double lane_dot_total(const ColsParams<double>& P, long c, double acc) { return spec_dot_line(P, c, acc); }
 
 template <class T, int NL, int NT, int MINB, int R0, int... Rs>
 __global__ void __launch_bounds__(NT, MINB) cols_fast_kernel(ColsParams<T> P) {
@@ -58,6 +78,9 @@
         ooff = (size_t)by * P.out_ostride + (size_t)bz * P.out_bstride + c0;
     };
 
+    const bool dot = mode == CM_FUSED && P.dot;
+    __shared__ double s_dot[NT / 32];
+
     if constexpr (NST == 1) {
         for (long t = blockIdx.x; t < ntiles; t += gridDim.x) {
             long c0; size_t ioff, ooff;
@@ -65,6 +88,7 @@
             const long nvalid = P.inner - c0;
             const cplx<T>* in = P.in + ioff;
             cplx<T>* out = P.out + ooff;
+            double dsum = 0.0;
             for (int lane = tid; lane < NL; lane += NT) {
                 if ((long)lane * LPT >= nvalid) continue;
                 const int rows_in = mode == CM_INV ? Ln : P.n_in;
@@ -74,7 +98,12 @@
                 for (int r = 0; r < R0; ++r)
                     v[r] = r < rows_in ? lane_from_global(in + cols_rowoff<T>(r, P.pitch, P.in_split_len, P.in_split_stride) + lane * LPT) : lzero<T>();
                 if (mode != CM_INV) lbfly<R0, false, T>(v);
-                if (mode == CM_FUSED) {
+                if (dot) {
+                    typename LaneAcc<T>::type acc{};
+#pragma unroll
+                    for (int r = 0; r < R0; ++r) v[r] = lane_spec_dot(v[r], lane_real_ldg(reinterpret_cast<const T*>(P.spec), (size_t)r * spitch + c0 + lane * LPT), acc);
+                    dsum += lane_dot_total(P, c0 + lane * LPT, acc);
+                } else if (mode == CM_FUSED) {
 #pragma unroll
                     for (int r = 0; r < R0; ++r) v[r] = lane_spec(v[r], P.spec, P.spec_kind, (size_t)r * spitch + c0 + lane * LPT);
                 }
@@ -82,6 +111,17 @@
 #pragma unroll
                 for (int r = 0; r < R0; ++r)
                     if (r < rows_out) lane_to_global(out + cols_rowoff<T>(r, P.pitch, P.out_split_len, P.out_split_stride) + lane * LPT, v[r]);
+            }
+            if (dot) {
+                spec_dot_warp(dsum, s_dot, tid);
+                __syncthreads();
+                if (tid < 32) {
+                    int b, ti;
+                    spec_dot_tile(P, t, b, ti);
+                    const unsigned done = spec_dot_publish(P.st, s_dot, NT / 32, (long)b * P.nx * P.ny + ti, b, tid);
+                    spec_dot_finish(P.st, P.dot - 1, done, b, P.nx * P.ny, tid);
+                }
+                __syncthreads();
             }
         }
         return;
@@ -182,7 +222,9 @@
                 if (spec_smem) { cp_async_wait_all(); __syncthreads(); }
             }
 
+            unsigned dot_done = 0;
             {
+                double dsum = 0.0;
 #pragma unroll 2
                 for (int it = tid; it < (Ln / RLAST) * NL; it += NT) {
                     const int lane = it % NL, bf = it / NL;
@@ -199,7 +241,19 @@
                         for (int r = 0; r < RLAST; ++r) v[r] = base[r * NL];
                         lbfly<RLAST, false, T>(v);
                     }
-                    if (mode == CM_FUSED) {
+                    if (dot) {
+                        typename LaneAcc<T>::type acc{};
+                        if (spec_smem) {
+                            const unsigned char* sp = side + ((size_t)sslot(p0) * NL + lane) * SPEC_LANE;
+#pragma unroll
+                            for (int r = 0; r < RLAST; ++r) v[r] = lane_spec_dot(v[r], lane_real_ld((const T*)nullptr, sp + r * NL * SPEC_LANE), acc);
+                        } else if (ok) {
+                            const size_t sidx = (size_t)p0 * spitch + c0 + lane * LPT;
+#pragma unroll
+                            for (int r = 0; r < RLAST; ++r) v[r] = lane_spec_dot(v[r], lane_real_ldg(reinterpret_cast<const T*>(P.spec), sidx + (size_t)r * spitch), acc);
+                        }
+                        dsum += lane_dot_total(P, c0 + lane * LPT, acc);
+                    } else if (mode == CM_FUSED) {
                         if (spec_smem) {
                             const unsigned char* sp = side + ((size_t)sslot(p0) * NL + lane) * SPEC_LANE;
 #pragma unroll
@@ -222,7 +276,13 @@
                         for (int r = 0; r < RLAST; ++r) base[r * NL] = v[r];
                     }
                 }
+                if (dot) spec_dot_warp(dsum, s_dot, tid);
                 __syncthreads();
+                if (dot && tid < 32) {
+                    int b, ti;
+                    spec_dot_tile(P, t, b, ti);
+                    dot_done = spec_dot_publish(P.st, s_dot, NT / 32, (long)b * P.nx * P.ny + ti, b, tid);
+                }
             }
             if (stage_in && t + gridDim.x < ntiles) prefetch_input(t + gridDim.x);
             if (mode == CM_FWD) continue;
@@ -253,6 +313,11 @@
                         }
                     }
                 }
+            }
+            if (dot && tid < 32) {
+                int b, ti;
+                spec_dot_tile(P, t, b, ti);
+                spec_dot_finish(P.st, P.dot - 1, dot_done, b, P.nx * P.ny, tid);
             }
         }
     }
@@ -650,7 +715,7 @@
     HIPGP_DYN_SMEM(smem_raw);
     Lane<T>* s = reinterpret_cast<Lane<T>*>(smem_raw);
     const int tid = threadIdx.x;
-    if (P.mode != RI_PLAIN && P.st.flags[0]) return;
+    if (P.st.flags && P.st.flags[0]) return;
     const long g0 = (long)blockIdx.x * NROW;
     const long g1 = g0 + NROW < P.total_rows ? g0 + NROW : P.total_rows;
     const int nl = (int)(g1 - g0);
diff --git a/hipgp_b200/csrc/plan.cu b/hipgp_b200/csrc/plan.cu
--- a/hipgp_b200/csrc/plan.cu
+++ b/hipgp_b200/csrc/plan.cu
@@ -137,6 +137,7 @@
     const long P = g.P;
     const int* done = gated ? st.flags : nullptr;
     const bool fast = geom_allows_fast(g);
+    auto fused_dot = [&](ColsParams<T>& C) { C.dot = fi.dot; C.st = st; C.dot_P = P; C.dot_H = g.H; };
 
     long rows_in = 1, rows_out = 1;
     for (int d = 0; d + 1 < D; ++d) { rows_in *= n_in[d]; rows_out *= n_out[d]; }
@@ -155,6 +156,7 @@
         C.in = W1; C.out = W1; C.n_in = n_in[0]; C.n_out = n_out[0]; C.inner = g.H + 1; C.pitch = P;
         C.in_ostride = C.out_ostride = 0; C.in_bstride = C.out_bstride = Wrows * P;
         C.f = g.fcol[0].dev; C.mode = CM_FUSED; C.spec = spec; C.spec_kind = spec_kind; C.done_flag = done;
+        fused_dot(C);
         launch_cols<T>(pl, C, 1, B, s, fast);
     } else if (D == 3) {
         const long R0 = std::max(n_in[0], n_out[0]);
@@ -168,14 +170,17 @@
         C.in = W2; C.out = W2; C.n_in = n_in[0]; C.n_out = n_out[0]; C.inner = L1 * P; C.pitch = L1 * P;
         C.in_ostride = C.out_ostride = 0; C.in_bstride = C.out_bstride = R0 * L1 * P;
         C.f = g.fcol[0].dev; C.mode = CM_FUSED; C.spec = spec; C.spec_kind = spec_kind;
+        fused_dot(C);
         launch_cols<T>(pl, C, 1, B, s, fast);
+        C.dot = 0;
         C.in = W2; C.out = W1; C.n_in = n_out[1]; C.n_out = n_out[1]; C.inner = g.H + 1; C.pitch = P;
         C.in_ostride = L1 * P; C.in_bstride = R0 * L1 * P; C.out_ostride = (long)n_out[1] * P; C.out_bstride = Wrows * P;
         C.f = g.fcol[1].dev; C.mode = CM_INV; C.spec = nullptr; C.spec_kind = SPEC_NONE;
         launch_cols<T>(pl, C, n_out[0], B, s, fast);
     }
 
-    R.out = (T*)fi.out; R.v0 = (T*)fi.v0; R.mode = fi.mode; R.dot_kind = fi.dot_kind;
+    R.out = (T*)fi.out; R.v0 = (T*)fi.v0;
+    R.mode = (D == 1 && fi.dot) ? RI_DOT : RI_PLAIN; R.dot_kind = fi.dot - 1;
     R.total_rows = B * rows_out; R.nrows = (int)rows_out; R.n_real = n_out[D - 1];
     if (D == 1) { R.spec = spec; R.spec_kind = spec_kind; }
     launch_rows<T>(pl, true, R, s, fast);
@@ -195,6 +200,12 @@
     long grp = (long)(budget_mb * 1048576.0 / per_rhs);
     (void)pl;
     return std::max<long>(1, std::min<long>(B, grp));
+}
+
+template <class T>
+static long partial_per_rhs(const Geom<T>& g, long rows) {
+    const long lines = g.D == 2 ? (long)g.H + 1 : (g.D == 3 ? (long)g.L[1] * g.P : 0);
+    return std::max(rows, lines);
 }
 
 template <class T>
@@ -216,7 +227,7 @@
             s2.zr = st.zr + b0; s2.zr_prev = st.zr_prev + b0; s2.pAp = st.pAp + b0; s2.rr = st.rr + b0;
             s2.rr_all = st.rr_all ? st.rr_all : st.rr;
             s2.row_cnt = st.row_cnt + b0;
-            s2.partial = st.partial + b0 * std::max(rows_in, rows_out);
+            s2.partial = st.partial + b0 * partial_per_rhs(g, std::max(rows_in, rows_out));
         }
         run_pipeline_group<T>(pl, g, n_in, n_out, spec, spec_kind, nb, f2, i2, s2, gated, s);
     }
@@ -429,7 +440,7 @@
     if (B == 0) return;
     if (!in || !out) throw Error("null vector pointer");
     RowsFusion ff, fi;
-    ff.mode = RF_PLAIN; ff.in = in; fi.mode = RI_PLAIN; fi.out = out;
+    ff.mode = RF_PLAIN; ff.in = in; fi.out = out;
     const bool wide = (mode == HIPGP_MV_RT || mode == HIPGP_MV_R);
     if (wide) ensure_wide<T>(pl, s);
     Geom<T>& g = geom(pl, wide, Tag<T>());
@@ -455,7 +466,7 @@
     long nrows = 1;
     for (int d = 0; d + 1 < pl->D; ++d) nrows *= pl->m[d];
     for (DevBuf* b : {&pl->vr, &pl->vp, &pl->vz, &pl->vAp}) b->ensure(sizeof(T) * (size_t)(B * M), &pl->dev_bytes);
-    pl->partial.ensure(sizeof(double) * (size_t)(B * nrows), &pl->dev_bytes);
+    pl->partial.ensure(sizeof(double) * (size_t)(B * partial_per_rhs(geom(pl, false, Tag<T>()), nrows)), &pl->dev_bytes);
     pl->scal.ensure(sizeof(double) * (size_t)(4 * B), &pl->dev_bytes);
     const bool fresh = pl->cnt.bytes < sizeof(unsigned) * (size_t)(B + 1);
     pl->cnt.ensure(sizeof(unsigned) * (size_t)(B + 1), &pl->dev_bytes);
@@ -507,7 +518,7 @@
     CK(cudaMemsetAsync(reinterpret_cast<char*>(st.flags) + 2 * sizeof(int), 1, 1, s));
     RowsFusion ff, fi;
     if (precond) {
-        ff.mode = RF_PLAIN; ff.in = r; fi.mode = RI_DOT; fi.dot_kind = DOT_ZR; fi.out = z; fi.v0 = r;
+        ff.mode = RF_PLAIN; ff.in = r; fi.dot = 1 + DOT_ZR; fi.out = z; fi.v0 = r;
         run_pipeline<T>(pl, g, nn, nn, pl->specCinv.p, SPEC_REAL, B, ff, fi, st, false, s);
     } else {
         launch_vec<T>(pl, RF_SELFDOT, st, B, r, nullptr, nullptr, nullptr, s);
@@ -530,12 +541,12 @@
     for (int c = 0; c < niter; ++c) {
         ff = RowsFusion(); fi = RowsFusion();
         ff.mode = RF_PUPDATE; ff.in = z; ff.v0 = p;
-        fi.mode = RI_DOT; fi.dot_kind = DOT_PAP; fi.out = Ap; fi.v0 = p;
+        fi.dot = 1 + DOT_PAP; fi.out = Ap; fi.v0 = p;
         run_pipeline<T>(pl, g, nn, nn, pl->specK.p, SPEC_REAL, B, ff, fi, st, true, s);
         if (precond) {
             ff = RowsFusion(); fi = RowsFusion();
             ff.mode = RF_XRUPDATE; ff.in = Ap; ff.v0 = r; ff.v1 = x; ff.v2 = p;
-            fi.mode = RI_DOT; fi.dot_kind = DOT_ZR; fi.out = z; fi.v0 = r;
+            fi.dot = 1 + DOT_ZR; fi.out = z; fi.v0 = r;
             run_pipeline<T>(pl, g, nn, nn, pl->specCinv.p, SPEC_REAL, B, ff, fi, st, true, s);
         } else {
             launch_vec<T>(pl, RF_XRUPDATE, st, B, Ap, r, x, p, s);
diff --git a/hipgp_b200/csrc/plan_types.cuh b/hipgp_b200/csrc/plan_types.cuh
--- a/hipgp_b200/csrc/plan_types.cuh
+++ b/hipgp_b200/csrc/plan_types.cuh
@@ -239,7 +239,8 @@
 };
 
 struct RowsFusion {
-    int mode = 0, dot_kind = 0, do_fft = 1;
+    int mode = 0, do_fft = 1;
+    int dot = 0;
     const void* in = nullptr; void* out = nullptr; void* v0 = nullptr; void* v1 = nullptr; const void* v2 = nullptr;
 };
 
```

Result: slower. 424.9, median of 6 (-5.9%).
